# KubiakJakub01/Valle2

Measured on AMD Instinct MI355X. Metric: acoustic tokens/sec (AR decode), higher is better.
Workload: dtype f32; 1 GPU; configs[1]: 12-layer/512-dim AR decoder greedy generate, batch 32, 1024-token prompt -> 512 new tokens, 1xMI355X per rank; rows_per_gpu=32

## Files before the change

### include/valle_hip.h

```cpp
#ifndef VALLE_HIP_H
#define VALLE_HIP_H

#include <stddef.h>
#include <stdint.h>

#ifdef __cplusplus
extern "C" {
#endif

#define VH_VERSION 135
#define VH_MAX_TABLES 32
#define VH_SAMPLE_MAX_V 16384
#define VH_HEAD_DIM 64

enum { VH_OK = 0, VH_EINVAL = -1, VH_EALIGN = -2, VH_EUNSUPPORTED = -3, VH_ELAUNCH = -4,
       VH_ESTATE = -5 };

enum { VH_ACT_NONE = 0, VH_ACT_GELU_ERF = 1,
       VH_ACT_GELU_BWD = 2,
       VH_ACT_GELU_ERF_D = 3,
       VH_ACT_MUL = 4          };

enum {
    VH_MASK_FULL = 0,
    VH_MASK_PREFIX = 1,
    VH_MASK_EXPLICIT = 2
};

int vh_version(void);
const char* vh_last_error(void);

enum { VH_TUNE_DECODE_VARIANT = 0,
       VH_TUNE_DECODE_WAVES = 1,
       VH_TUNE_ROW_GROUPS = 2,
       VH_TUNE_TILE_DMA = 4,
       VH_TUNE_REDUCE_BLOCK = 3,
       VH_TUNE_FFN_FUSED = 5,
       VH_TUNE_GRAPH_STEPS = 6,
       VH_TUNE_FFN_SLICE = 7,
       VH_TUNE_FFN_ROWS = 8,
       VH_TUNE_LN_STATS = 9,
       VH_TUNE_TAIL_SPLIT = 10,
       VH_TUNE_TN_WGS = 11,
       VH_TUNE_DECODE_COMBINE = 12,
       VH_TUNE_ATTN_BWD = 13,
       VH_TUNE_ATTN_BWD_CHUNKS = 14,
       VH_TUNE_BF16_GEMM = 15,
       VH_TUNE_COUNT = 16 };
int vh_set_tuning(int knob, int value);

typedef struct { uint64_t seed; uint64_t site; float p; } vh_dropout_spec;
int vh_dropout(const float* x, int ldx, float* out, int ldo, int64_t rows, int cols, const vh_dropout_spec* spec,
               void* stream);
int vh_dropout_mask(uint8_t* keep, int64_t rows, int cols, const vh_dropout_spec* spec, void* stream);

enum { VH_DEVERR_EMBED_ID = 1, VH_DEVERR_TARGET = 2 };
int vh_embed_sum_pe(const int64_t* ids, int64_t ids_bstride, int64_t ids_tstride,
                    int64_t ids_jstride, const float* const* tables, const int32_t* vocab, int n_tables,
                    const float* pe, int pos0, const int32_t* lens, float* out,
                    int64_t out_bstride, int out_t0, int B, int T, int d, int32_t* err_flag,
                    const int32_t* row_pos0, const int32_t* row_t0, const vh_dropout_spec* drop, void* stream);

int vh_add_pe(const float* x, const float* pe, float* out, int B, int T, int d, int pos0, void* stream);

int vh_layernorm(const float* x, const float* gamma, const float* beta, const float* ada_scale,
                 const float* ada_shift, float* out, int rows, int d, float eps, void* stream);

int vh_linear(const float* A, int lda, const float* W, const float* bias, const float* residual,
              int ldr, float* out, int ldo, int M, int N, int K, int act, const float* ln_gamma,
              const float* ln_beta, const float* ada_scale, const float* ada_shift, float ln_eps,
              void* stream);

size_t vh_linear_ws_bytes(int M, int N, int K);
int vh_linear_ws(const float* A, int lda, const float* W, const float* bias, const float* residual,
                 int ldr, float* out, int ldo, int M, int N, int K, int act, void* workspace,
                 size_t workspace_bytes, void* stream);

int vh_linear_qkv(const float* A, int lda, const float* Wqkv, float* q_out, int ldq, float* kcache,
                  float* vcache, const int32_t* cache_len, int B, int T, int d_model, int n_heads,
                  int S_max, const float* ln_gamma, const float* ln_beta, const float* ada_scale,
                  const float* ada_shift, float ln_eps, void* stream);
// ... 150 lines not shown
    float *x;
    float *q, *attn, *hidden, *logits;
    void *attn_partial;
    void *gemm_ws;
    size_t gemm_ws_bytes;
    int32_t *cache_len, *audio_pos, *eos_count;
    const int32_t *pos_base;
    int64_t *codes;
    int64_t codes_stride;
    int top_k;
    float top_p, temperature;
    uint64_t seed;
    float *sum_logprobs;
    void *ffn_ws;
    size_t ffn_ws_bytes;
    int kv_bf16;
    int prefix_len, prefix_S;
    size_t attn_partial_bytes;
    void *head_ws;
    size_t head_ws_bytes;
    const uint64_t *seed_dev;
    const uint16_t *proj_w16;
    int n_groups, beams_per_group, prefix_cap;
    const int32_t *prefix_lens;
    const vh_row_sampling *row_sampling;
} vh_ar_decoder_desc;

typedef struct vh_ar_decoder vh_ar_decoder;
vh_ar_decoder* vh_ar_decoder_create(const vh_ar_decoder_desc* desc);
void vh_ar_decoder_destroy(vh_ar_decoder* dec);
int vh_ar_decoder_step(vh_ar_decoder* dec, void* stream);
int vh_ar_decoder_capture(vh_ar_decoder* dec, void* stream);
int vh_ar_decoder_replay(vh_ar_decoder* dec, int n_steps, void* stream);
int vh_ar_decoder_profile_attn(vh_ar_decoder* dec, int n_steps, void* stream, float* mean_ms,
                               float* floor_ms, float* kernel_ms);

int vh_layernorm_bwd(const float* x, const float* gamma, const float* beta, const float* ada_scale,
                     const float* dy, float* dx, float* dgamma, float* dbeta, float* dscale,
                     float* dshift, const float* dres, float* dcolsum, float* dx_drop, const vh_dropout_spec* drop,
                     int rows, int d, float eps, void* stream);
int vh_gelu(const float* pre, const float* dh, float* out, int64_t n, void* stream);
int vh_softmax_rows(float* S, int ld, int B, int n_heads, int Tq, int Tk, float scale, int mode,
                    int x_len, const int32_t* x_len_dev, const int32_t* kv_len, const uint8_t* mask,
                    const uint8_t* pad, void* stream);
int vh_softmax_bwd(const float* P, float* dP, int ld, int64_t rows, int Tk, float scale, void* stream);
int vh_cross_entropy(const float* logits, int ld, int V, const int64_t* target, float* loss,
                     float* dlogits, int ldd, int rows, int32_t* err_flag, void* stream);
int vh_embed_bwd(const int64_t* ids, int64_t ids_bstride, int64_t ids_tstride, const float* dout,
                 int64_t dout_bstride, int out_t0, float* dtable, int vocab, int B, int T, int d,
                 int32_t* err_flag, const vh_dropout_spec* drop, void* stream);
int vh_colsum(const float* x, int ld, float* out, int rows, int cols, void* stream);

typedef struct { const float* w; const float* b; float* dw; float* db; } vh_adaproj_item;
int vh_adaproj_fwd(const vh_adaproj_item* items, int n, const float* emb, float* out, int N, int K, void* stream);
int vh_adaproj_bwd(const vh_adaproj_item* items, int n, const float* emb, const float* dout, float* demb, int N, int K,
                   void* stream);

int vh_categorical_rows(const float* logits, int ld, int V, int rows, float temperature, int greedy,
                        uint64_t seed, uint32_t stream_id, int64_t* tokens, int64_t tokens_stride,
                        float* logprob, void* stream);

size_t vh_adamw_ws_bytes(void);
int vh_adamw_flat(float* param, float* grad, float* exp_avg, float* exp_avg_sq, int64_t n, float lr,
                  float beta1, float beta2, float eps, float weight_decay, int step, float grad_scale,
                  float max_norm, int zero_grad, void* workspace, float* norm_out, const int32_t* block_slot,
                  const int32_t* slot_step, const int32_t* guard, void* stream);

size_t vh_linear_ex_ws_bytes(int M, int N, int K);
int vh_linear_ex(const float* A, int lda, const float* W, const float* bias, const float* residual, int ldr,
                 float* out, int ldo, float* pre_out, int ldp, float* dcolsum, int M, int N, int K, int act,
                 const vh_dropout_spec* drop, void* workspace, size_t workspace_bytes, void* stream);

int vh_transpose(const float* in, int ldi, int rows, int cols, float* out, int ldo, void* stream);
typedef struct { const float* in; float* out; int32_t ldi, rows, cols, ldo, tile0, pad_; } vh_transpose_item;
int vh_transpose_many(const vh_transpose_item* items, int n, int total_tiles, void* stream);

size_t vh_gemm_tn_ws_bytes(int M, int NI, int NJ);
int vh_gemm_tn(const float* A, int lda, const float* B, int ldb, float* C, int ldc, int M, int NI, int NJ,
               void* workspace, size_t workspace_bytes, void* stream);

int vh_gemm_batched(const float* A, int lda, int64_t sAb, int64_t sAh, int a_kmajor, const float* B,
                    int ldb, int64_t sBb, int64_t sBh, int b_kmajor, float* C, int ldc, int64_t sCb,
                    int64_t sCh, int M, int N, int K, int batch, int H, int k_splits, void* stream);

typedef struct {
    int B, T, d_model, n_heads, dff, n_layers, S_max, mode, x_len;
    float ln_eps;
    const vh_layer* layers;
    const float* ada;
    const int32_t *x_len_dev, *kv_len;
    const uint8_t *mask, *pad;
    float *x, *xn, *q, *attn, *hidden;
    void *gemm_ws;
    size_t gemm_ws_bytes;
    const float *x_in;
} vh_forward_desc;
int vh_transformer_forward(const vh_forward_desc* desc, void* stream);

int vh_h16_format(void);
int vh_to_bf16(const float* src, int64_t lds, uint16_t* dst, int64_t ldd, int64_t rows, int cols, void* stream);
int vh_layernorm_bf16(const float* x, const float* gamma, const float* beta, const float* ada_scale,
                      const float* ada_shift, uint16_t* out, int rows, int d, float eps, void* stream);
int vh_linear_bf16(const uint16_t* A, int lda, const uint16_t* W, const float* bias, const float* residual, int ldr,
                   void* out, int ldo, int out_bf16, int M, int N, int K, int act, void* stream);
int vh_linear_qkv_bf16(const uint16_t* A, int lda, const uint16_t* Wqkv, uint16_t* q_out, int ldq, uint16_t* kcache16,
                       uint16_t* vcache16, const int32_t* cache_len, int B, int T, int d_model, int n_heads, int S_max,
                       void* stream);
int vh_attn_rows_bf16(const uint16_t* q, int ldq, const uint16_t* kcache16, const uint16_t* vcache16, uint16_t* out, int ldo,
                      int B, int n_heads, int Tq, int Tk, int S_max, int mode, int x_len, const int32_t* x_len_dev,
                      const int32_t* kv_len, void* stream);

typedef struct { const uint16_t *wqkv, *wo, *w1, *w2; uint16_t *kcache16, *vcache16; } vh_layer16;
typedef struct {
    int B, T, d_model, n_heads, dff, n_layers, S_max, mode, x_len;
    float ln_eps;
    const vh_layer* layers;
    const vh_layer16* layers16;
    const float* ada;
    const int32_t *x_len_dev, *kv_len;
    float* x;
    const float* x_in;
    uint16_t *xn16, *q16, *attn16, *hidden16;
} vh_forward16_desc;
int vh_transformer_forward_bf16(const vh_forward16_desc* desc, void* stream);

#ifdef __cplusplus
}
#endif
// ... 2 lines not shown
```

### valle2_amd/_lib.py

```python
from __future__ import annotations

import ctypes as C
import os
from pathlib import Path

import torch

_HERE = Path(__file__).resolve().parent
LIB_PATH = _HERE / 'csrc' / 'libvalle_hip.so'

c_f32p = C.c_void_p
c_i32p = C.c_void_p
c_i64p = C.c_void_p
c_u8p = C.c_void_p


class VhError(RuntimeError):
    pass


class VhDropoutSpec(C.Structure):
    _fields_ = [('seed', C.c_uint64), ('site', C.c_uint64), ('p', C.c_float)]


# ... 12 lines not shown
        'wqkv_f16', 'wo16', 'w1_f16', 'w2_16')]


class VhArDecoderDesc(C.Structure):
    _fields_ = [
        ('B', C.c_int), ('d_model', C.c_int), ('n_heads', C.c_int), ('dff', C.c_int),
        ('n_layers', C.c_int), ('S_max', C.c_int), ('V', C.c_int), ('eos', C.c_int),
        ('n_split', C.c_int), ('ln_eps', C.c_float),
        ('layers', C.POINTER(VhLayer)),
        ('proj_w', C.c_void_p), ('audio_emb', C.c_void_p), ('audio_pe', C.c_void_p),
        ('x', C.c_void_p), ('q', C.c_void_p), ('attn', C.c_void_p), ('hidden', C.c_void_p),
        ('logits', C.c_void_p), ('attn_partial', C.c_void_p), ('gemm_ws', C.c_void_p),
        ('gemm_ws_bytes', C.c_size_t),
        ('cache_len', C.c_void_p), ('audio_pos', C.c_void_p), ('eos_count', C.c_void_p),
        ('pos_base', C.c_void_p), ('codes', C.c_void_p), ('codes_stride', C.c_int64),
        ('top_k', C.c_int), ('top_p', C.c_float), ('temperature', C.c_float), ('seed', C.c_uint64),
        ('sum_logprobs', C.c_void_p), ('ffn_ws', C.c_void_p), ('ffn_ws_bytes', C.c_size_t), ('kv_bf16', C.c_int),
        ('prefix_len', C.c_int), ('prefix_S', C.c_int), ('attn_partial_bytes', C.c_size_t),
        ('head_ws', C.c_void_p), ('head_ws_bytes', C.c_size_t), ('seed_dev', C.c_void_p), ('proj_w16', C.c_void_p),
        ('n_groups', C.c_int), ('beams_per_group', C.c_int), ('prefix_cap', C.c_int), ('prefix_lens', C.c_void_p),
        ('row_sampling', C.c_void_p),
    ]


class VhForwardDesc(C.Structure):
    _fields_ = [
        ('B', C.c_int), ('T', C.c_int), ('d_model', C.c_int), ('n_heads', C.c_int),
        ('dff', C.c_int), ('n_layers', C.c_int), ('S_max', C.c_int), ('mode', C.c_int),
        ('x_len', C.c_int), ('ln_eps', C.c_float),
        ('layers', C.POINTER(VhLayer)), ('ada', C.c_void_p),
        ('x_len_dev', C.c_void_p), ('kv_len', C.c_void_p), ('mask', C.c_void_p), ('pad', C.c_void_p),
        ('x', C.c_void_p), ('xn', C.c_void_p), ('q', C.c_void_p), ('attn', C.c_void_p),
        ('hidden', C.c_void_p), ('gemm_ws', C.c_void_p), ('gemm_ws_bytes', C.c_size_t), ('x_in', C.c_void_p),
    ]


class VhLayer16(C.Structure):
    _fields_ = [(n, C.c_void_p) for n in ('wqkv', 'wo', 'w1', 'w2', 'kcache16', 'vcache16')]


class VhForward16Desc(C.Structure):
    _fields_ = [
        ('B', C.c_int), ('T', C.c_int), ('d_model', C.c_int), ('n_heads', C.c_int),
        ('dff', C.c_int), ('n_layers', C.c_int), ('S_max', C.c_int), ('mode', C.c_int),
        ('x_len', C.c_int), ('ln_eps', C.c_float),
        ('layers', C.POINTER(VhLayer)), ('layers16', C.POINTER(VhLayer16)), ('ada', C.c_void_p),
        ('x_len_dev', C.c_void_p), ('kv_len', C.c_void_p), ('x', C.c_void_p), ('x_in', C.c_void_p),
        ('xn16', C.c_void_p), ('q16', C.c_void_p), ('attn16', C.c_void_p), ('hidden16', C.c_void_p),
    ]


SIGNATURES = {
    'vh_version': (C.c_int, []),
    'vh_last_error': (C.c_char_p, []),
    'vh_set_tuning': (C.c_int, [C.c_int, C.c_int]),
    'vh_embed_sum_pe': (C.c_int, [c_i64p, C.c_int64, C.c_int64, C.c_int64, C.POINTER(C.c_void_p),
                                  C.POINTER(C.c_int32), C.c_int, c_f32p, C.c_int, c_i32p, c_f32p, C.c_int64,
                                  C.c_int, C.c_int, C.c_int, C.c_int, c_i32p, c_i32p, c_i32p, c_dropp, C.c_void_p]),
    'vh_dropout': (C.c_int, [c_f32p, C.c_int, c_f32p, C.c_int, C.c_int64, C.c_int, c_dropp, C.c_void_p]),
    'vh_dropout_mask': (C.c_int, [c_u8p, C.c_int64, C.c_int, c_dropp, C.c_void_p]),
    'vh_add_pe': (C.c_int, [c_f32p, c_f32p, c_f32p, C.c_int, C.c_int, C.c_int, C.c_int, C.c_void_p]),
    'vh_layernorm': (C.c_int, [c_f32p, c_f32p, c_f32p, c_f32p, c_f32p, c_f32p, C.c_int, C.c_int,
                               C.c_float, C.c_void_p]),
    'vh_linear': (C.c_int, [c_f32p, C.c_int, c_f32p, c_f32p, c_f32p, C.c_int, c_f32p, C.c_int,
                            C.c_int, C.c_int, C.c_int, C.c_int, c_f32p, c_f32p, c_f32p, c_f32p,
                            C.c_float, C.c_void_p]),
# ... 59 lines not shown
    'vh_kv_store': (C.c_int, [c_f32p, C.c_int, c_f32p, c_f32p, C.c_int, C.c_int, C.c_int, C.c_int, C.c_int, C.c_void_p]),
    'vh_greedy_step': (C.c_int, [c_f32p, C.c_int, C.c_int, C.c_int, c_i64p, C.c_int64, c_i32p,
                                 c_i32p, c_f32p, c_f32p, c_i32p, c_i32p, c_f32p, C.c_int, C.c_int,
                                 C.c_void_p]),
    'vh_decode_groups_poll': (C.c_int, [c_i64p, C.c_int64, C.c_int, c_i32p, c_i32p, c_i32p, C.c_int, C.c_int, C.c_int, C.c_int,
                                        c_i32p, c_i32p, c_i32p, C.c_void_p]),
    'vh_decode_group_reset': (C.c_int, [c_i64p, C.c_int64, C.c_int, c_i64p, C.c_int, C.c_int, C.c_int, C.c_int, C.c_int, C.c_int,
                                        C.c_int, c_i32p, c_i32p, c_i32p, c_f32p, c_i32p, C.c_void_p]),
    'vh_head_greedy_ws_bytes': (C.c_size_t, [C.c_int, C.c_int]),
    'vh_head_greedy': (C.c_int, [c_f32p, C.c_int, c_f32p, c_f32p, C.c_int, C.c_int, C.c_int, c_i64p, C.c_int64, c_i32p,
                                 c_i32p, c_f32p, c_f32p, c_i32p, c_i32p, c_f32p, C.c_int, C.c_int, C.c_void_p, C.c_size_t,
                                 C.c_void_p]),
    'vh_sample_step': (C.c_int, [c_f32p, C.c_int, C.c_int, C.c_int, C.c_int, C.c_float, C.c_float, C.c_uint64,
                                 c_i64p, C.c_int64, c_i32p, c_i32p, c_f32p, c_f32p, c_f32p, c_i32p, c_i32p,
                                 c_f32p, C.c_int, C.c_int, C.c_void_p]),
    'vh_sample_step_wide': (C.c_int, [c_f32p, C.c_int, C.c_int, C.c_int, C.c_int, C.c_float, C.c_float, C.c_uint64,
                                      c_i64p, C.c_int64, c_i32p, c_i32p, c_f32p, c_f32p, c_f32p, c_i32p, c_i32p,
                                      c_f32p, C.c_int, C.c_int, C.c_void_p]),
    'vh_sample_step_rows': (C.c_int, [c_f32p, C.c_int, C.c_int, C.c_int, C.c_void_p, c_i64p, C.c_int64, c_i32p, c_i32p,
                                      c_f32p, c_f32p, c_f32p, c_i32p, c_i32p, c_f32p, C.c_int, C.c_int, C.c_void_p]),
    'vh_sample_step_wide_rows': (C.c_int, [c_f32p, C.c_int, C.c_int, C.c_int, C.c_void_p, c_i64p, C.c_int64, c_i32p, c_i32p,
                                           c_f32p, c_f32p, c_f32p, c_i32p, c_i32p, c_f32p, C.c_int, C.c_int, C.c_void_p]),
    'vh_categorical_rows': (C.c_int, [c_f32p, C.c_int, C.c_int, C.c_int, C.c_float, C.c_int, C.c_uint64, C.c_uint32,
                                      c_i64p, C.c_int64, c_f32p, C.c_void_p]),
    'vh_adamw_ws_bytes': (C.c_size_t, []),
    'vh_adamw_flat': (C.c_int, [c_f32p, c_f32p, c_f32p, c_f32p, C.c_int64, C.c_float, C.c_float, C.c_float,
                                C.c_float, C.c_float, C.c_int, C.c_float, C.c_float, C.c_int, C.c_void_p,
                                c_f32p, c_i32p, c_i32p, c_i32p, C.c_void_p]),
    'vh_ar_decoder_create': (C.c_void_p, [C.POINTER(VhArDecoderDesc)]),
    'vh_ar_decoder_destroy': (None, [C.c_void_p]),
    'vh_ar_decoder_step': (C.c_int, [C.c_void_p, C.c_void_p]),
    'vh_ar_decoder_capture': (C.c_int, [C.c_void_p, C.c_void_p]),
    'vh_ar_decoder_replay': (C.c_int, [C.c_void_p, C.c_int, C.c_void_p]),
    'vh_ar_decoder_profile_attn': (C.c_int, [C.c_void_p, C.c_int, C.c_void_p,
                                             C.POINTER(C.c_float), C.POINTER(C.c_float), C.POINTER(C.c_float)]),
    'vh_layernorm_bwd': (C.c_int, [c_f32p, c_f32p, c_f32p, c_f32p, c_f32p, c_f32p, c_f32p, c_f32p, c_f32p,
                                   c_f32p, c_f32p, c_f32p, c_f32p, c_dropp, C.c_int, C.c_int, C.c_float, C.c_void_p]),
    'vh_gelu': (C.c_int, [c_f32p, c_f32p, c_f32p, C.c_int64, C.c_void_p]),
    'vh_softmax_rows': (C.c_int, [c_f32p, C.c_int, C.c_int, C.c_int, C.c_int, C.c_int, C.c_float, C.c_int,
                                  C.c_int, c_i32p, c_i32p, c_u8p, c_u8p, C.c_void_p]),
    'vh_softmax_bwd': (C.c_int, [c_f32p, c_f32p, C.c_int, C.c_int64, C.c_int, C.c_float, C.c_void_p]),
    'vh_cross_entropy': (C.c_int, [c_f32p, C.c_int, C.c_int, c_i64p, c_f32p, c_f32p, C.c_int, C.c_int,
                                   c_i32p, C.c_void_p]),
    'vh_embed_bwd': (C.c_int, [c_i64p, C.c_int64, C.c_int64, c_f32p, C.c_int64, C.c_int, c_f32p, C.c_int,
                               C.c_int, C.c_int, C.c_int, c_i32p, c_dropp, C.c_void_p]),
    'vh_colsum': (C.c_int, [c_f32p, C.c_int, c_f32p, C.c_int, C.c_int, C.c_void_p]),
    'vh_linear_ex': (C.c_int, [c_f32p, C.c_int, c_f32p, c_f32p, c_f32p, C.c_int, c_f32p, C.c_int, c_f32p, C.c_int,
                               c_f32p, C.c_int, C.c_int, C.c_int, C.c_int, c_dropp, C.c_void_p, C.c_size_t, C.c_void_p]),
    'vh_linear_ex_ws_bytes': (C.c_size_t, [C.c_int, C.c_int, C.c_int]),
    'vh_transpose': (C.c_int, [c_f32p, C.c_int, C.c_int, C.c_int, c_f32p, C.c_int, C.c_void_p]),
    'vh_transpose_many': (C.c_int, [C.c_void_p, C.c_int, C.c_int, C.c_void_p]),
    'vh_adaproj_fwd': (C.c_int, [C.c_void_p, C.c_int, c_f32p, c_f32p, C.c_int, C.c_int, C.c_void_p]),
    'vh_adaproj_bwd': (C.c_int, [C.c_void_p, C.c_int, c_f32p, c_f32p, c_f32p, C.c_int, C.c_int, C.c_void_p]),
    'vh_gemm_tn_ws_bytes': (C.c_size_t, [C.c_int, C.c_int, C.c_int]),
    'vh_gemm_tn': (C.c_int, [c_f32p, C.c_int, c_f32p, C.c_int, c_f32p, C.c_int, C.c_int, C.c_int, C.c_int,
                             C.c_void_p, C.c_size_t, C.c_void_p]),
    'vh_gemm_batched': (C.c_int, [c_f32p, C.c_int, C.c_int64, C.c_int64, C.c_int, c_f32p, C.c_int, C.c_int64,
                                  C.c_int64, C.c_int, c_f32p, C.c_int, C.c_int64, C.c_int64, C.c_int, C.c_int,
                                  C.c_int, C.c_int, C.c_int, C.c_int, C.c_void_p]),
    'vh_transformer_forward': (C.c_int, [C.POINTER(VhForwardDesc), C.c_void_p]),
    'vh_h16_format': (C.c_int, []),
    'vh_to_bf16': (C.c_int, [c_f32p, C.c_int64, C.c_void_p, C.c_int64, C.c_int64, C.c_int, C.c_void_p]),
    'vh_layernorm_bf16': (C.c_int, [c_f32p, c_f32p, c_f32p, c_f32p, c_f32p, C.c_void_p, C.c_int, C.c_int, C.c_float,
                                    C.c_void_p]),
    'vh_linear_bf16': (C.c_int, [C.c_void_p, C.c_int, C.c_void_p, c_f32p, c_f32p, C.c_int, C.c_void_p, C.c_int, C.c_int,
                                 C.c_int, C.c_int, C.c_int, C.c_int, C.c_void_p]),
    'vh_linear_qkv_bf16': (C.c_int, [C.c_void_p, C.c_int, C.c_void_p, C.c_void_p, C.c_int, C.c_void_p, C.c_void_p, c_i32p,
                                     C.c_int, C.c_int, C.c_int, C.c_int, C.c_int, C.c_void_p]),
    'vh_attn_rows_bf16': (C.c_int, [C.c_void_p, C.c_int, C.c_void_p, C.c_void_p, C.c_void_p, C.c_int, C.c_int, C.c_int,
                                    C.c_int, C.c_int, C.c_int, C.c_int, C.c_int, c_i32p, c_i32p, C.c_void_p]),
    'vh_transformer_forward_bf16': (C.c_int, [C.POINTER(VhForward16Desc), C.c_void_p]),
}

_lib = None


def load_library(path: os.PathLike | None = None) -> C.CDLL:
    p = Path(path or LIB_PATH)
    if not p.exists():
        raise VhError(f'{p} not found: build it with `python __graft_entry__.py build` '
                      f'(make -C valle2_amd/csrc). There is no CPU fallback.')
    lib = C.CDLL(str(p))
    for name, (res, args) in SIGNATURES.items():
        fn = getattr(lib, name)
        fn.restype = res
        fn.argtypes = args
    raw_set = lib.vh_set_tuning

    def set_tuning(knob, value):
        global TUNING_EPOCH
        TUNING_EPOCH += 1
        return raw_set(knob, value)
    lib.vh_set_tuning = set_tuning
    return lib


TUNING_EPOCH = 0


def h16_dtype():
    global _H16
    if _H16 is None:
        _H16 = torch.bfloat16 if load_library().vh_h16_format() else torch.float16
    return _H16


_H16 = None


def lib() -> C.CDLL:
    global _lib
    if _lib is None:
        if not torch.cuda.is_available():
            raise VhError('valle2_amd needs a HIP device (MI355X): torch.cuda.is_available() is '
                          'False and there is no CPU fallback. The CPU oracle lives in oracle/ and '
                          'is test infrastructure only.')
        _lib = load_library()
        n = sum(1 for line in open('/proc/self/maps') if 'libamdhip64' in line and ' r-xp ' in line)
        if n > 1:
            raise VhError('two HIP runtimes are mapped in this process; import torch before '
                          'loading libvalle_hip.so')
    return _lib


def check(rc: int, what: str = ''):
    if rc != 0:
        msg = lib().vh_last_error()
        raise VhError(f'{what} failed ({rc}): {msg.decode() if msg else ""}')


# ... 85 lines not shown
```

### valle2_amd/csrc/attention.hip

```cpp
#include <hip/hip_ext.h>
#include "vh_common.h"
#include <mutex>
#include <queue>
#include <type_traits>
#include <unordered_map>
#include <vector>

#define HD VH_HEAD_DIM
#define LOG2E 1.44269504088896340736f
#define NEG_INF (-INFINITY)

#define PART_LD 72

typedef uint32_t u32x4 __attribute__((ext_vector_type(4)));
__device__ __forceinline__ u32x4 ld16_stream(const uint16_t* p) {
    return __builtin_nontemporal_load(reinterpret_cast<const u32x4*>(p));
}
__device__ __forceinline__ float row8_sum(float v) {
    v += dpp_get<0xB1, 0xF>(v, 0.f);
    v += dpp_get<0x4E, 0xF>(v, 0.f);
    v += dpp_get<0x141, 0xF>(v, 0.f);
    return v;
}
#define BF_LO(w) vh_h16_lo(w)
// ... 465 lines not shown
    const bool fused_combine = n_split > 1 && (combine_knob == 1 || (combine_knob == 0 && n_split == 2));
    unsigned* arrived = fused_combine ? (unsigned*)((char*)partial + decode_records_bytes(B, n_heads, n_split)) : nullptr;
    if (variant != 1 && big && n_split == 1 && nw == 0) {
        const int waves = 8;
        hipExtLaunchKernelGGL((attn_decode_ring_kernel<8, 2>), grid, dim3(waves * 64), 0, s, g_attn_ev[0], g_attn_ev[1], 0, q,
                              ldq, kcache, vcache, out, ldo, cache_len, len_bias, n_heads, S_max);
    } else {
        const int waves = nw ? nw : (big ? 16 : 4);
        if (waves == 16) AD(attn_decode_kernel, 16); else if (waves == 8) AD(attn_decode_kernel, 8);
        else AD(attn_decode_kernel, 4);
    }
#undef AD
    if (n_split > 1 && !fused_combine)
        hipLaunchKernelGGL(attn_decode_combine_kernel, dim3(B * n_heads), dim3(64), 0, s,
                           (const float*)partial, out, ldo, n_heads, n_split);
    VH_CHECK_LAUNCH("vh_attn_decode");
    return VH_OK;
}

#define QB 128
#define KT 32
#define KLD 68

struct RowsArgs {
    const float* q; int ldq;
    const float* kc; const float* vc;
    float* out; int ldo;
    int n_heads, Tq, Tk, S_max, mode, x_len;
    const int32_t* x_len_dev; const int32_t* kv_len;
    const uint8_t* mask; const uint8_t* pad;
    int n_qblocks;
    float* lse2;
    int64_t mask_bstride;
};

__global__ __launch_bounds__(256, 2) void attn_rows_kernel(RowsArgs a) {
    __shared__ __attribute__((aligned(16))) float lds[2 * 2 * KT * KLD];
    const int tid = threadIdx.x, lane = tid & 63, w = tid >> 6;
    const int r = lane & 31, h = lane >> 5;
    const int n_bh = gridDim.x / a.n_qblocks;
    const int bh = blockIdx.x % n_bh, b = bh / a.n_heads, head = bh - b * a.n_heads;
    const int q0 = (a.n_qblocks - 1 - (int)(blockIdx.x / n_bh)) * QB;
    const int q_off = a.Tk - a.Tq;
    const int kvl = a.kv_len ? min(a.kv_len[b], a.Tk) : a.Tk;
    const int xl = a.x_len_dev ? a.x_len_dev[b] : a.x_len;

    const int last_pos = q_off + min(q0 + QB, a.Tq) - 1;
    int kmax = kvl;
    if (a.mode == VH_MASK_PREFIX) kmax = min(kvl, max(xl, last_pos >= xl ? last_pos + 1 : 0));
    if (a.mode == VH_MASK_EXPLICIT) kmax = a.Tk;
    const int n_tiles = (kmax + KT - 1) / KT;

    const int qi = q0 + w * 32 + r;
    const int qpos = q_off + qi;
    const float qscale = 0.125f * LOG2E;
    f32x4 qf[8];
    {
        const float* qp = a.q + ((int64_t)b * a.Tq + qi) * a.ldq + head * HD + 4 * h;
#pragma unroll
        for (int t = 0; t < 8; ++t)
            qf[t] = qi < a.Tq ? ld4(qp + 8 * t) * qscale : f32x4{0.f, 0.f, 0.f, 0.f};
    }

    const float* kb = a.kc + (int64_t)bh * a.S_max * HD;
    const float* vb = a.vc + (int64_t)bh * a.S_max * HD;
    const int skey = tid >> 4, squad = (tid & 15) * 4;
    f32x4 rk[2], rv[2];
    auto gload = [&](int k0) {
#pragma unroll
        for (int i = 0; i < 2; ++i) {
            const uint32_t off = (uint32_t)(min(k0 + skey + 16 * i, a.Tk - 1) * HD + squad) * 4u;
            rk[i] = ld4((const float*)((const char*)kb + off));
            rv[i] = ld4((const float*)((const char*)vb + off));
        }
    };
// ... 84 lines not shown
            }
#pragma unroll
            for (int e = 0; e < 16; ++e) {
                const float* vrow = vs + ((e & 3) + 8 * (e >> 2) + 4 * h) * KLD + r;
                O0 = __builtin_amdgcn_mfma_f32_32x32x2f32(vrow[0], S[e], O0, 0, 0, 0);
                O1 = __builtin_amdgcn_mfma_f32_32x32x2f32(vrow[32], S[e], O1, 0, 0, 0);
            }
        }
        if (kt + 1 < n_tiles) lstore(cur ^ 1);
        __syncthreads();
    }

    const float ltot = l + __shfl_xor(l, 32, 64);
    const float inv = 1.0f / ltot;
    if (a.lse2 && h == 0 && qi < a.Tq) a.lse2[(int64_t)bh * a.Tq + qi] = m + log2f(ltot);
    float* ob = lds;
#pragma unroll
    for (int g4 = 0; g4 < 4; ++g4) {
        f32x4 v0 = {O0[4 * g4], O0[4 * g4 + 1], O0[4 * g4 + 2], O0[4 * g4 + 3]};
        f32x4 v1 = {O1[4 * g4], O1[4 * g4 + 1], O1[4 * g4 + 2], O1[4 * g4 + 3]};
        st4(ob + (w * 32 + r) * KLD + 8 * g4 + 4 * h, v0 * inv);
        st4(ob + (w * 32 + r) * KLD + 32 + 8 * g4 + 4 * h, v1 * inv);
    }
    __syncthreads();
#pragma unroll
    for (int i = 0; i < 8; ++i) {
        const int row = skey + 16 * i;
        if (q0 + row < a.Tq)
            st4(a.out + ((int64_t)b * a.Tq + q0 + row) * a.ldo + head * HD + squad,
                ld4(ob + row * KLD + squad));
    }
}

static int attn_rows_launch(const float* q, int ldq, const float* kcache, const float* vcache,
                            float* out, int ldo, int B, int n_heads, int Tq, int Tk, int S_max,
                            int mode, int x_len, const int32_t* x_len_dev, const int32_t* kv_len,
                            const uint8_t* mask, const uint8_t* pad, float* lse2, void* stream, int64_t mask_bstride = 0) {
    VH_REQUIRE(q && kcache && vcache && out, VH_EINVAL, "vh_attn_rows: null pointer");
    VH_REQUIRE(B >= 0 && n_heads > 0 && Tq >= 0 && Tk >= Tq && S_max >= Tk, VH_EINVAL,
               "vh_attn_rows: bad dims B=%d h=%d Tq=%d Tk=%d S_max=%d", B, n_heads, Tq, Tk, S_max);
    VH_REQUIRE(mode == VH_MASK_FULL || mode == VH_MASK_PREFIX || mode == VH_MASK_EXPLICIT, VH_EINVAL,
               "vh_attn_rows: mode=%d", mode);
    VH_REQUIRE(mode != VH_MASK_EXPLICIT || mask, VH_EINVAL, "vh_attn_rows: explicit mode needs mask");
    VH_REQUIRE(ldq % 4 == 0 && ldo % 4 == 0 && ldq >= n_heads * HD && ldo >= n_heads * HD, VH_EINVAL,
               "vh_attn_rows: ldq=%d ldo=%d", ldq, ldo);
    VH_REQUIRE(vh_aligned16(q) && vh_aligned16(kcache) && vh_aligned16(vcache) && vh_aligned16(out),
               VH_EALIGN, "vh_attn_rows: pointers must be 16-byte aligned");
    if (B == 0 || Tq == 0) return VH_OK;
    const int nqb = (Tq + QB - 1) / QB;
    RowsArgs a{q, ldq, kcache, vcache, out, ldo, n_heads, Tq, Tk, S_max, mode, x_len,
               x_len_dev, kv_len, mask, pad, nqb, lse2, mask_bstride};
    dim3 grid(nqb * B * n_heads);
    hipLaunchKernelGGL(attn_rows_kernel, grid, dim3(256), 0, (hipStream_t)stream, a);
    VH_CHECK_LAUNCH("vh_attn_rows");
    return VH_OK;
}

extern "C" int vh_attn_rows(const float* q, int ldq, const float* kcache, const float* vcache,
                            float* out, int ldo, int B, int n_heads, int Tq, int Tk, int S_max,
                            int mode, int x_len, const int32_t* x_len_dev, const int32_t* kv_len,
                            const uint8_t* mask, const uint8_t* pad, void* stream) {
    return attn_rows_launch(q, ldq, kcache, vcache, out, ldo, B, n_heads, Tq, Tk, S_max, mode, x_len,
                            x_len_dev, kv_len, mask, pad, nullptr, stream);
}

extern "C" int vh_attn_rows_bmask(const float* q, int ldq, const float* kcache, const float* vcache, float* out, int ldo, int B,
                                  int n_heads, int Tq, int Tk, int S_max, const uint8_t* mask, int64_t mask_batch_stride,
                                  const uint8_t* pad, void* stream) {
    VH_REQUIRE(mask && (mask_batch_stride == 0 || mask_batch_stride >= (int64_t)Tq * Tk), VH_EINVAL,
               "vh_attn_rows_bmask: a (B,Tq,Tk) mask with batch stride >= Tq*Tk (or 0: one mask for every row), got %lld",
               (long long)mask_batch_stride);
    return attn_rows_launch(q, ldq, kcache, vcache, out, ldo, B, n_heads, Tq, Tk, S_max, VH_MASK_EXPLICIT, 0, nullptr, nullptr,
                            mask, pad, nullptr, stream, mask_batch_stride);
}

extern "C" int vh_attn_rows_lse(const float* q, int ldq, const float* kcache, const float* vcache,
                                float* out, int ldo, int B, int n_heads, int Tq, int Tk, int S_max,
                                int mode, int x_len, const int32_t* x_len_dev, const int32_t* kv_len,
                                const uint8_t* mask, const uint8_t* pad, float* lse2, void* stream) {
    VH_REQUIRE(lse2, VH_EINVAL, "vh_attn_rows_lse: null lse2");
    return attn_rows_launch(q, ldq, kcache, vcache, out, ldo, B, n_heads, Tq, Tk, S_max, mode, x_len,
                            x_len_dev, kv_len, mask, pad, lse2, stream);
}

struct BwdArgs {
    const float* q; int ldq;
    const float* kc; const float* vc;
    const float* o; int ldo;
// ... 1020 lines not shown
```

### valle2_amd/csrc/elementwise.hip

```cpp
#include "vh_common.h"

template <int CAP>
struct TablePtrs {
    const float* t[CAP];
    int vocab[CAP];
};

template <int CAP>
__global__ __launch_bounds__(256) void embed_sum_pe_kernel(
    const int64_t* __restrict__ ids, int64_t ids_bs, int64_t ids_ts, int64_t ids_js, TablePtrs<CAP> tabs,
    int n_tables, const float* __restrict__ pe, int pos0, const int32_t* __restrict__ lens,
    float* __restrict__ out, int64_t out_bs, int out_t0, int T, int d, int32_t* __restrict__ err_flag,
    const int32_t* __restrict__ row_pos0, const int32_t* __restrict__ row_t0, DropArgs drop) {
    const int lane = threadIdx.x & 63;
    const int t = blockIdx.x * 4 + (threadIdx.x >> 6);
    const int b = blockIdx.y;
    if (t >= T) return;
    if (lens && t >= lens[b]) return;
    if (row_pos0) pos0 = row_pos0[b];
    if (row_t0) out_t0 = row_t0[b];
    const int64_t* idp = ids + b * ids_bs + t * ids_ts;
    int64_t row[CAP];
    bool bad = false;
    for (int j = 0; j < n_tables; ++j) {
// ... 216 lines not shown
            if (ada_scale) y = ld4(ada_scale + c) * y + ld4(ada_shift + c);
            st4(orow + c, y);
        }
    }
}

extern "C" int vh_layernorm(const float* x, const float* gamma, const float* beta,
                            const float* ada_scale, const float* ada_shift, float* out, int rows,
                            int d, float eps, void* stream) {
    VH_REQUIRE(x && gamma && beta && out, VH_EINVAL, "vh_layernorm: null pointer");
    VH_REQUIRE((ada_scale == nullptr) == (ada_shift == nullptr), VH_EINVAL,
               "vh_layernorm: ada_scale and ada_shift must be given together");
    VH_REQUIRE(rows >= 0 && d > 0 && d % 4 == 0 && d <= 4096, VH_EINVAL,
               "vh_layernorm: bad dims rows=%d d=%d (d multiple of 4, <= 4096)", rows, d);
    VH_REQUIRE(vh_aligned16(x) && vh_aligned16(out) && vh_aligned16(gamma) && vh_aligned16(beta) &&
                   vh_aligned16(ada_scale) && vh_aligned16(ada_shift),
               VH_EALIGN, "vh_layernorm: pointers must be 16-byte aligned");
    if (rows == 0) return VH_OK;
    dim3 grid((rows + 3) / 4), block(256);
    hipStream_t s = (hipStream_t)stream;
#define LN_LAUNCH(NV)                                                                            \
    hipLaunchKernelGGL(layernorm_kernel<NV>, grid, block, 0, s, x, gamma, beta, ada_scale,       \
                       ada_shift, out, rows, d, eps)
    if (d <= 256) LN_LAUNCH(1);
    else if (d <= 512) LN_LAUNCH(2);
    else if (d <= 1024) LN_LAUNCH(4);
    else if (d <= 2048) LN_LAUNCH(8);
    else LN_LAUNCH(16);
#undef LN_LAUNCH
    VH_CHECK_LAUNCH("vh_layernorm");
    return VH_OK;
}

__global__ __launch_bounds__(256) void greedy_step_kernel(
    const float* __restrict__ logits, int ldl, int V, int eos, int64_t* __restrict__ codes,
    int64_t codes_stride, int32_t* __restrict__ eos_count, const int32_t* __restrict__ pos_base,
    const float* __restrict__ audio_emb, const float* __restrict__ pe,
    int32_t* __restrict__ audio_pos, int32_t* __restrict__ cache_len, float* __restrict__ x_next, int d) {
    __shared__ float s_val[4];
    __shared__ int s_idx[4];
    __shared__ int s_tok;
    const int b = blockIdx.x;
    const int tid = threadIdx.x, lane = tid & 63, w = tid >> 6;
    const float* lr = logits + (int64_t)b * ldl;
    float best = -INFINITY;
    int bi = 0x7fffffff;
    for (int i = tid; i < V; i += 256) {
        const float v = lr[i];
        if (v > best || (v == best && i < bi)) { best = v; bi = i; }
    }
#pragma unroll
    for (int o = 32; o > 0; o >>= 1) {
        const float ov = __shfl_xor(best, o, 64);
        const int oi = __shfl_xor(bi, o, 64);
        if (ov > best || (ov == best && oi < bi)) { best = ov; bi = oi; }
    }
    if (lane == 0) { s_val[w] = best; s_idx[w] = bi; }
    __syncthreads();
    const int pos = audio_pos[b];
    if (tid == 0) {
        for (int k = 1; k < 4; ++k)
            if (s_val[k] > best || (s_val[k] == best && s_idx[k] < bi)) { best = s_val[k]; bi = s_idx[k]; }
        int64_t* row = codes + (int64_t)b * codes_stride;
        int tok = bi;
        if (row[pos - 1] == (int64_t)eos) tok = eos;
        row[pos] = tok;
        if (tok == eos) atomicAdd(&eos_count[pos - (pos_base ? pos_base[b] : 0)], 1);
        s_tok = tok;
    }
    __syncthreads();
    const int tok = s_tok;
    const float* er = audio_emb + (int64_t)tok * d;
    const float* pr = pe + (int64_t)pos * d;
    for (int c = tid * 4; c < d; c += 1024) {
        const f32x4 e = ld4(er + c) + ld4(pr + c);
        st4(x_next + (int64_t)b * d + c, e);
    }
    if (tid == 0) {
        audio_pos[b] = pos + 1;
        cache_len[b] += 1;
    }
}

extern "C" int vh_greedy_step(const float* logits, int ldl, int V, int eos, int64_t* codes,
                              int64_t codes_stride, int32_t* eos_count, const int32_t* pos_base,
                              const float* audio_emb, const float* pe, int32_t* audio_pos,
                              int32_t* cache_len, float* x_next, int B, int d, void* stream) {
    VH_REQUIRE(logits && codes && eos_count && audio_emb && pe && audio_pos && cache_len && x_next,
               VH_EINVAL, "vh_greedy_step: null pointer");
    VH_REQUIRE(B > 0 && V > 0 && ldl >= V && d > 0 && d % 4 == 0, VH_EINVAL,
               "vh_greedy_step: bad dims B=%d V=%d ldl=%d d=%d", B, V, ldl, d);
    VH_REQUIRE(vh_aligned16(audio_emb) && vh_aligned16(pe) && vh_aligned16(x_next), VH_EALIGN,
               "vh_greedy_step: audio_emb/pe/x_next must be 16-byte aligned");
    hipLaunchKernelGGL(greedy_step_kernel, dim3(B), dim3(256), 0, (hipStream_t)stream, logits, ldl,
                       V, eos, codes, codes_stride, eos_count, pos_base, audio_emb, pe, audio_pos,
                       cache_len, x_next, d);
    VH_CHECK_LAUNCH("vh_greedy_step");
    return VH_OK;
}

#define SAMPLE_MAXV 2048

__device__ __forceinline__ float uniform01(uint64_t seed, uint32_t row, uint32_t pos) {
    uint64_t z = seed + 0x9E3779B97F4A7C15ull * (((uint64_t)row << 32) | (uint64_t)(pos + 1u));
    z = (z ^ (z >> 30)) * 0xBF58476D1CE4E5B9ull;
    z = (z ^ (z >> 27)) * 0x94D049BB133111EBull;
    z ^= z >> 31;
    return (float)(z >> 40) * (1.0f / 16777216.0f);
}

__device__ __forceinline__ uint32_t okey(float x) {
    const uint32_t u = __float_as_uint(x);
    return (u & 0x80000000u) ? ~u : (u | 0x80000000u);
}

#define ROW_SAMPLING_LOAD(rec)                                            \
    do {                                                                  \
        const vh_row_sampling r_ = (rec);                                 \
        seed = r_.seed;                                                   \
        draw_key = r_.key;                                                \
        top_k = r_.top_k;                                                 \
        top_p = r_.top_p;                                                 \
        inv_temp = 1.0f / r_.temperature;                                 \
        greedy = top_k == 1;                                              \
        if (greedy) { top_p = 1.0f; inv_temp = 1.0f; }                    \
    } while (0)

__global__ __launch_bounds__(256) void sample_step_kernel(
    const float* __restrict__ logits, int ldl, int V, int eos, int top_k, float top_p, float inv_temp,
    uint64_t seed, int64_t* __restrict__ codes, int64_t codes_stride, int32_t* __restrict__ eos_count,
    const int32_t* __restrict__ pos_base, float* __restrict__ sum_logprobs,
    const float* __restrict__ audio_emb, const float* __restrict__ pe, int32_t* __restrict__ audio_pos,
    int32_t* __restrict__ cache_len, float* __restrict__ x_next, int d, int npow2, const uint64_t* __restrict__ seed_dev,
    const vh_row_sampling* __restrict__ rs) {
    uint32_t draw_key = blockIdx.x;
    bool greedy = false;
    if (rs) {
        ROW_SAMPLING_LOAD(rs[blockIdx.x]);
    } else if (seed_dev) {
        seed += *seed_dev;
    }
    __shared__ float s_val[SAMPLE_MAXV];
    __shared__ int s_idx[SAMPLE_MAXV];
    __shared__ int s_hist[256];
    __shared__ int s_sel[4];
    __shared__ float s_red[8];
    __shared__ int s_tok;
    const int b = blockIdx.x, tid = threadIdx.x, lane = tid & 63, wv = tid >> 6;
    const float* lr = logits + (int64_t)b * ldl;
    const int pos = audio_pos[b];
    int pick_tok = 0;
    float pick_logprob = 0.f;

    const bool fast = top_k > 0 && top_k < V && top_p == 1.0f;
    if (fast) {
        float vmax = -INFINITY;
        for (int i = tid; i < V; i += 256) {
            float x = lr[i] * inv_temp;
            if (greedy) x += 0.0f;
            s_val[i] = x;
            vmax = fmaxf(vmax, x);
        }
        vmax = wave_max(vmax);
        if (lane == 0) s_red[wv] = vmax;
        uint32_t prefix = 0, mask = 0;
        int want = top_k;
        for (int shift = 24; shift >= 0; shift -= 8) {
// ... 118 lines not shown
                float tail = 0.f;
                int n2 = n_keep;
                while (n2 > 1) {
                    tail += expf(s_val[n2 - 1] - m);
                    if (tail > limit) break;
                    --n2;
                }
                n_keep = n2;
                total = 0.f;
                for (int i = 0; i < n_keep; ++i) total += expf(s_val[i] - m);
            }
            const float u = uniform01(seed, draw_key, (uint32_t)pos) * total;
            float acc = 0.f;
            int pick = n_keep - 1;
            for (int i = 0; i < n_keep; ++i) {
                acc += expf(s_val[i] - m);
                if (acc > u) { pick = i; break; }
            }
            s_sel[2] = s_idx[pick];
            s_red[4] = (s_val[pick] - m) - logf(total);
        }
        __syncthreads();
        pick_tok = s_sel[2];
        pick_logprob = s_red[4];
    }
    if (greedy) pick_logprob = 0.f;
    if (tid == 0) {
        int64_t* row = codes + (int64_t)b * codes_stride;
        int tok = pick_tok;
        const bool finished = row[pos - 1] == (int64_t)eos;
        if (sum_logprobs && !finished) sum_logprobs[b] += pick_logprob;
        if (finished) tok = eos;
        row[pos] = tok;
        if (tok == eos) atomicAdd(&eos_count[pos - (pos_base ? pos_base[b] : 0)], 1);
        s_tok = tok;
    }
    __syncthreads();
    const int tok = s_tok;
    const float* er = audio_emb + (int64_t)tok * d;
    const float* pr = pe + (int64_t)pos * d;
    for (int c = tid * 4; c < d; c += 1024) {
        const f32x4 e = ld4(er + c) + ld4(pr + c);
        st4(x_next + (int64_t)b * d + c, e);
    }
    if (tid == 0) {
        audio_pos[b] = pos + 1;
        cache_len[b] += 1;
    }
}

int vh_internal_sample_step(const float* logits, int ldl, int V, int eos, int top_k, float top_p,
                            float temperature, uint64_t seed, const uint64_t* seed_dev, const vh_row_sampling* rs, int64_t* codes, int64_t codes_stride,
                            int32_t* eos_count, const int32_t* pos_base, float* sum_logprobs,
                            const float* audio_emb, const float* pe, int32_t* audio_pos,
                            int32_t* cache_len, float* x_next, int B, int d, void* stream) {
    VH_REQUIRE(logits && codes && eos_count && audio_emb && pe && audio_pos && cache_len && x_next,
               VH_EINVAL, "vh_sample_step: null pointer");
    VH_REQUIRE(B > 0 && V > 0 && V <= SAMPLE_MAXV && ldl >= V && d > 0 && d % 4 == 0, VH_EINVAL,
               "vh_sample_step: bad dims B=%d V=%d (<= %d) ldl=%d d=%d", B, V, SAMPLE_MAXV, ldl, d);
    VH_REQUIRE(rs || temperature > 0.f, VH_EINVAL, "vh_sample_step: temperature must be positive");
    VH_REQUIRE(vh_aligned16(rs), VH_EALIGN, "vh_sample_step: the per-row sampling records must be 16-byte aligned");
    VH_REQUIRE(vh_aligned16(audio_emb) && vh_aligned16(pe) && vh_aligned16(x_next), VH_EALIGN,
               "vh_sample_step: audio_emb/pe/x_next must be 16-byte aligned");
    int npow2 = 2;
    while (npow2 < V) npow2 <<= 1;
    hipLaunchKernelGGL(sample_step_kernel, dim3(B), dim3(256), 0, (hipStream_t)stream, logits, ldl, V,
                       eos, top_k, top_p, rs ? 1.0f : 1.0f / temperature, seed, codes, codes_stride, eos_count,
                       pos_base, sum_logprobs, audio_emb, pe, audio_pos, cache_len, x_next, d, npow2, seed_dev, rs);
    VH_CHECK_LAUNCH("vh_sample_step");
    return VH_OK;
}

extern "C" int vh_sample_step(const float* logits, int ldl, int V, int eos, int top_k, float top_p,
                              float temperature, uint64_t seed, int64_t* codes, int64_t codes_stride,
                              int32_t* eos_count, const int32_t* pos_base, float* sum_logprobs,
                              const float* audio_emb, const float* pe, int32_t* audio_pos,
                              int32_t* cache_len, float* x_next, int B, int d, void* stream) {
    return vh_internal_sample_step(logits, ldl, V, eos, top_k, top_p, temperature, seed, nullptr, nullptr, codes, codes_stride, eos_count,
                                   pos_base, sum_logprobs, audio_emb, pe, audio_pos, cache_len, x_next, B, d, stream);
}

extern "C" int vh_sample_step_rows(const float* logits, int ldl, int V, int eos, const vh_row_sampling* rs, int64_t* codes,
                                  int64_t codes_stride, int32_t* eos_count, const int32_t* pos_base, float* sum_logprobs,
                                  const float* audio_emb, const float* pe, int32_t* audio_pos, int32_t* cache_len,
                                  float* x_next, int B, int d, void* stream) {
    VH_REQUIRE(rs, VH_EINVAL, "vh_sample_step_rows: null sampling records (vh_sample_step takes one filter for every row)");
    return vh_internal_sample_step(logits, ldl, V, eos, 0, 1.f, 1.f, 0, nullptr, rs, codes, codes_stride, eos_count, pos_base, sum_logprobs,
                                  audio_emb, pe, audio_pos, cache_len, x_next, B, d, stream);
}

#define WIDE_THREADS 1024
#define WIDE_WAVES (WIDE_THREADS / 64)
#define WIDE_PER (VH_SAMPLE_MAX_V / WIDE_THREADS)

template <typename T>
__device__ __forceinline__ T wide_block_scan(T v, T* s_w, T* excl, T* total) {
    const int lane = threadIdx.x & 63, wv = threadIdx.x >> 6;
    T incl = v;
#pragma unroll
    for (int o = 1; o < 64; o <<= 1) {
        const T up = __shfl_up(incl, o, 64);
// ... 15 lines not shown
    return before + incl;
}

__device__ __forceinline__ void wide_draw(const float* s_val, int n, float m, float u01, float* s_w, int* s_out,
                                          float* s_tot) {
    const int tid = threadIdx.x;
    const int per = (n + WIDE_THREADS - 1) / WIDE_THREADS;
    const int j0 = min(n, tid * per), j1 = min(n, j0 + per);
    float s = 0.f;
    for (int j = j0; j < j1; ++j) s += expf(s_val[j] - m);
    if (tid == 0) s_out[0] = n - 1;
    float excl, total;
    const float incl = wide_block_scan(s, s_w, &excl, &total);
    const float u = u01 * total;
    if (j1 > j0 && excl <= u && incl > u) {
        float acc = excl;
        int pick = j1 - 1;
        for (int j = j0; j < j1; ++j) {
            acc += expf(s_val[j] - m);
            if (acc > u) { pick = j; break; }
        }
        s_out[0] = pick;
    }
    if (tid == 0) s_tot[0] = total;
    __syncthreads();
}

__global__ __launch_bounds__(WIDE_THREADS) void sample_step_wide_kernel(
    const float* __restrict__ logits, int ldl, int V, int eos, int top_k, float top_p, float inv_temp,
    uint64_t seed, int64_t* __restrict__ codes, int64_t codes_stride, int32_t* __restrict__ eos_count,
    const int32_t* __restrict__ pos_base, float* __restrict__ sum_logprobs,
    const float* __restrict__ audio_emb, const float* __restrict__ pe, int32_t* __restrict__ audio_pos,
    int32_t* __restrict__ cache_len, float* __restrict__ x_next, int d, const uint64_t* __restrict__ seed_dev,
    const vh_row_sampling* __restrict__ rs) {
    uint32_t draw_key = blockIdx.x;
    bool greedy = false;
    if (rs) {
        ROW_SAMPLING_LOAD(rs[blockIdx.x]);
    } else if (seed_dev) {
        seed += *seed_dev;
    }
    __shared__ float s_val[VH_SAMPLE_MAX_V];
    __shared__ int s_idx[VH_SAMPLE_MAX_V];
    __shared__ int s_hist[256];
    __shared__ float s_wf[WIDE_WAVES];
    __shared__ int s_wi[WIDE_WAVES];
    __shared__ float s_max[WIDE_WAVES];
    __shared__ int s_sel[3];
    __shared__ float s_tot;
    __shared__ int s_tok;
    const int b = blockIdx.x, tid = threadIdx.x, lane = tid & 63, wv = tid >> 6;
    const float* lr = logits + (int64_t)b * ldl;
    const int pos = audio_pos[b];

    float vmax = -INFINITY;
    for (int i = tid; i < V; i += WIDE_THREADS) {
        float x = lr[i] * inv_temp;
        if (greedy) x += 0.0f;
        s_val[i] = x;
        vmax = fmaxf(vmax, x);
    }
    vmax = wave_max(vmax);
    if (lane == 0) s_max[wv] = vmax;
    __syncthreads();
    float m = s_max[0];
#pragma unroll
    for (int w = 1; w < WIDE_WAVES; ++w) m = fmaxf(m, s_max[w]);
// ... 98 lines not shown
            }
        int n_keep = n;
        if (top_p >= 0.f && top_p <= 1.f) {
            const int run = (n + WIDE_THREADS - 1) / WIDE_THREADS;
            const int j1 = max(0, n - tid * run), j0 = max(0, j1 - run);
            float s = 0.f;
            for (int j = j1 - 1; j >= j0; --j) s += expf(s_val[j] - m);
            float after, total;
            wide_block_scan(s, s_wf, &after, &total);
            const float limit = (1.0f - top_p) * total;
            float tail = after;
            int over = 0;
            for (int j = j1 - 1; j >= j0; --j) {
                tail += expf(s_val[j] - m);
                over += j >= 1 && tail > limit;
            }
            int ex, n_over;
            wide_block_scan(over, s_wi, &ex, &n_over);
            n_keep = 1 + n_over;
        }
        wide_draw(s_val, n_keep, m, u01, s_wf, &s_sel[2], &s_tot);
    }
    const int slot = s_sel[2];
    const int pick_tok = s_idx[slot];
    const float pick_logprob = greedy ? 0.f : (s_val[slot] - m) - logf(s_tot);

    if (tid == 0) {
        int64_t* row = codes + (int64_t)b * codes_stride;
        int tok = pick_tok;
        const bool finished = row[pos - 1] == (int64_t)eos;
        if (sum_logprobs && !finished) sum_logprobs[b] += pick_logprob;
        if (finished) tok = eos;
        row[pos] = tok;
        if (tok == eos) atomicAdd(&eos_count[pos - (pos_base ? pos_base[b] : 0)], 1);
        s_tok = tok;
    }
    __syncthreads();
    const int tok = s_tok;
    const float* er = audio_emb + (int64_t)tok * d;
    const float* pr = pe + (int64_t)pos * d;
    for (int c = tid * 4; c < d; c += 4 * WIDE_THREADS) {
        const f32x4 e = ld4(er + c) + ld4(pr + c);
        st4(x_next + (int64_t)b * d + c, e);
    }
    if (tid == 0) {
        audio_pos[b] = pos + 1;
        cache_len[b] += 1;
    }
}

int vh_internal_sample_step_wide(const float* logits, int ldl, int V, int eos, int top_k, float top_p,
                                 float temperature, uint64_t seed, const uint64_t* seed_dev, const vh_row_sampling* rs, int64_t* codes,
                                 int64_t codes_stride, int32_t* eos_count, const int32_t* pos_base, float* sum_logprobs,
                                 const float* audio_emb, const float* pe, int32_t* audio_pos,
                                 int32_t* cache_len, float* x_next, int B, int d, void* stream) {
    VH_REQUIRE(logits && codes && eos_count && audio_emb && pe && audio_pos && cache_len && x_next,
               VH_EINVAL, "vh_sample_step_wide: null pointer");
    VH_REQUIRE(B > 0 && V > 0 && V <= VH_SAMPLE_MAX_V && ldl >= V && d > 0 && d % 4 == 0, VH_EINVAL,
               "vh_sample_step_wide: bad dims B=%d V=%d (<= %d) ldl=%d d=%d", B, V, VH_SAMPLE_MAX_V, ldl, d);
    VH_REQUIRE(rs || temperature > 0.f, VH_EINVAL, "vh_sample_step_wide: temperature must be positive");
    VH_REQUIRE(vh_aligned16(rs), VH_EALIGN, "vh_sample_step_wide: the per-row sampling records must be 16-byte aligned");
    VH_REQUIRE(vh_aligned16(audio_emb) && vh_aligned16(pe) && vh_aligned16(x_next), VH_EALIGN,
               "vh_sample_step_wide: audio_emb/pe/x_next must be 16-byte aligned");
    hipLaunchKernelGGL(sample_step_wide_kernel, dim3(B), dim3(WIDE_THREADS), 0, (hipStream_t)stream, logits, ldl, V,
                       eos, top_k, top_p, rs ? 1.0f : 1.0f / temperature, seed, codes, codes_stride, eos_count,
                       pos_base, sum_logprobs, audio_emb, pe, audio_pos, cache_len, x_next, d, seed_dev, rs);
    VH_CHECK_LAUNCH("vh_sample_step_wide");
    return VH_OK;
}

extern "C" int vh_sample_step_wide(const float* logits, int ldl, int V, int eos, int top_k, float top_p,
                                   float temperature, uint64_t seed, int64_t* codes, int64_t codes_stride,
                                   int32_t* eos_count, const int32_t* pos_base, float* sum_logprobs,
                                   const float* audio_emb, const float* pe, int32_t* audio_pos,
                                   int32_t* cache_len, float* x_next, int B, int d, void* stream) {
    return vh_internal_sample_step_wide(logits, ldl, V, eos, top_k, top_p, temperature, seed, nullptr, nullptr, codes, codes_stride,
                                        eos_count, pos_base, sum_logprobs, audio_emb, pe, audio_pos, cache_len, x_next, B, d,
                                        stream);
}

extern "C" int vh_sample_step_wide_rows(const float* logits, int ldl, int V, int eos, const vh_row_sampling* rs, int64_t* codes,
                                       int64_t codes_stride, int32_t* eos_count, const int32_t* pos_base, float* sum_logprobs,
                                       const float* audio_emb, const float* pe, int32_t* audio_pos, int32_t* cache_len,
                                       float* x_next, int B, int d, void* stream) {
    VH_REQUIRE(rs, VH_EINVAL, "vh_sample_step_wide_rows: null sampling records (vh_sample_step_wide takes one filter for every row)");
    return vh_internal_sample_step_wide(logits, ldl, V, eos, 0, 1.f, 1.f, 0, nullptr, rs, codes, codes_stride, eos_count, pos_base, sum_logprobs,
                                       audio_emb, pe, audio_pos, cache_len, x_next, B, d, stream);
}


__global__ __launch_bounds__(256) void categorical_rows_kernel(
    const float* __restrict__ logits, int ld, int V, int rows, float inv_temp, int greedy, uint64_t seed,
    uint32_t stream_id, int64_t* __restrict__ tokens, int64_t tokens_stride, float* __restrict__ logprob) {
    const int lane = threadIdx.x & 63;
    const int row = blockIdx.x * 4 + (threadIdx.x >> 6);
    if (row >= rows) return;
    const float* lr = logits + (int64_t)row * ld;
    const int chunk = (V + 63) / 64;
    const int i0 = min(V, lane * chunk), i1 = min(V, i0 + chunk);
// ... 185 lines not shown
```

### valle2_amd/csrc/gemm.hip

```cpp
#include <type_traits>

#include "vh_common.h"

struct GemmArgs {
    const float* A;
    int lda;
    const float* W;
    const float* bias;
    const float* res;
    int ldr;
    float* out;
    int ldo;
    int M, N, K, act;
    float* kc;
    float* vc;
    const int32_t* cache_len;
    int T, S_max, d_model, n_heads;
    float* aux;
    int ldx;
    float* colsum;
    int k_len;
    int rg_rows;
    int w16;
    DropArgs drop;
// ... 3 lines not shown
#endif
};

#ifdef VH_STAMPS
#define STAMP(k)                                                                         \
    do {                                                                                 \
        if (a.dbg && (threadIdx.x & 63) == 0)                                            \
            a.dbg[((int64_t)blockIdx.x * 16 + (threadIdx.x >> 6)) * 8 + (k)] = wall_clock64(); \
    } while (0)
#else
#define STAMP(k)
#endif

enum { EPI_PLAIN = 0, EPI_QKV = 1, EPI_PARTIAL = 2,
       EPI_QKV16 = 3 ,
       EPI_HEAD = 4  ,
       EPI_QKV_HD = 5  };
#define IS_QKV(E) ((E) == EPI_QKV || (E) == EPI_QKV16 || (E) == EPI_QKV_HD)

struct HeadStep {
    uint64_t* cand;
    int* counters;
    int V, eos;
    int64_t* codes;
    int64_t codes_stride;
    int32_t* eos_count;
    const int32_t* pos_base;
    const float* audio_emb;
    const float* pe;
    int32_t* audio_pos;
    int32_t* cache_len;
    float* x_next;
    int d;
};

__device__ __forceinline__ uint32_t vh_bf16_bits(float x) {
    const uint32_t u = __float_as_uint(x);
    return (u + 0x7fffu + ((u >> 16) & 1u)) >> 16;
}

template <int EPI>
__device__ __forceinline__ void store4(const GemmArgs& a, int m, int n, f32x4 v) {
    if (m >= a.M || n >= a.N) return;
    if (EPI == EPI_PARTIAL) {
        st4(a.out + ((int64_t)blockIdx.y * a.M + m) * a.ldo + n, v);
        return;
    }
    if (EPI == EPI_QKV) {
        const int which = n / a.d_model, c = n - which * a.d_model;
        if (which == 0) {
            st4(a.out + (int64_t)m * a.ldo + c, v);
        } else {
            const int head = c / VH_HEAD_DIM, e = c - head * VH_HEAD_DIM;
            const int b = m / a.T, t = m - b * a.T;
            const int pos = (a.cache_len ? a.cache_len[b] : 0) + t;
            float* base = which == 1 ? a.kc : a.vc;
            st4(base + (((int64_t)b * a.n_heads + head) * a.S_max + pos) * VH_HEAD_DIM + e, v);
        }
        return;
    }
    if (EPI == EPI_QKV_HD) {
        const int which = n / a.d_model, c = n - which * a.d_model;
        if (which == 0) {
            st4(a.out + (int64_t)m * a.ldo + c, v);
        } else {
            const int head = c / a.head_dim, e = c - head * a.head_dim;
// ... 278 lines not shown
                else if (a.act == VH_ACT_MUL) sv *= a.res[(int64_t)m * a.ldr + en + j];
                else if (a.res) sv += a.res[(int64_t)m * a.ldr + en + j];
                a.out[(int64_t)m * a.ldo + en + j] = sv;
            }
        }
    }
    if (EPI == EPI_PLAIN && a.colsum) tile_colsum(a, ct, csum, n0, tid);
}

template <int EPI>
__global__ __launch_bounds__(256, 2) void gemm_tile_kernel(GemmArgs a, int tiles_m, int tiles_n) {
    __shared__ __attribute__((aligned(16))) float lds[2][2][TM * LDS_LD];
    const int tid = threadIdx.x, lane = tid & 63, w = tid >> 6;
    const int r = lane & 31, h = lane >> 5;
    const int wm = w >> 1, wn = w & 1;

    const int nwg = tiles_m * tiles_n;
    const int bid = blockIdx.x;
    const int q8 = nwg / 8, r8 = nwg % 8, xcd = bid % 8;
    const int tile = (xcd < r8 ? xcd * (q8 + 1) : r8 * (q8 + 1) + (xcd - r8) * q8) + bid / 8;
    const int m0 = (tile / tiles_n) * TM, n0 = (tile % tiles_n) * TN;

    const int srow = tid >> 3, skq = (tid & 7) * 4;
    f32x4 ra[4], rw[4];
    const float* pa[4];
    const float* pw[4];
#pragma unroll
    for (int i = 0; i < 4; ++i) {
        const int row = srow + 32 * i;
        pa[i] = a.A + (int64_t)min(m0 + row, a.M - 1) * a.lda + skq + blockIdx.y * a.k_len;
        pw[i] = a.W + (int64_t)min(n0 + row, a.N - 1) * a.K + skq + blockIdx.y * a.k_len;
    }
    auto gload1 = [&](int i, int k0) {
        const int kk = k0 + skq < a.k_len ? k0 : 0;
        ra[i] = ld4(pa[i] + kk);
        rw[i] = ld4(pw[i] + kk);
    };
    auto gload = [&](int k0) {
#pragma unroll
        for (int i = 0; i < 4; ++i) gload1(i, k0);
    };
    auto lstore = [&](int buf, int k0) {
        const bool kin = k0 + skq < a.k_len;
#pragma unroll
        for (int i = 0; i < 4; ++i) {
            const int row = srow + 32 * i;
            st4(&lds[buf][0][row * LDS_LD + skq], kin ? ra[i] : f32x4{0.f, 0.f, 0.f, 0.f});
            st4(&lds[buf][1][row * LDS_LD + skq], kin ? rw[i] : f32x4{0.f, 0.f, 0.f, 0.f});
        }
    };

    f32x16 acc[2][2];
#pragma unroll
    for (int i = 0; i < 2; ++i)
#pragma unroll
        for (int j = 0; j < 2; ++j)
#pragma unroll
            for (int e = 0; e < 16; ++e) acc[i][j][e] = 0.f;

    const int nk = (a.k_len + TK - 1) / TK;
    gload(0);
    lstore(0, 0);

    TileEpi epi;
    tile_prefetch<EPI>(a, m0, n0, tid, epi);
    __syncthreads();
    f32x4 fa[2][2], fw[2][2];
// ... 15 lines not shown
            if (t < 3) fload((t + 1) & 1, cur, t + 1);
            __builtin_amdgcn_sched_barrier(0);
#pragma unroll
            for (int j = 0; j < 4; ++j) {
                acc[0][0] = __builtin_amdgcn_mfma_f32_32x32x2f32(fa[t & 1][0][j], fw[t & 1][0][j], acc[0][0], 0, 0, 0);
                acc[0][1] = __builtin_amdgcn_mfma_f32_32x32x2f32(fa[t & 1][0][j], fw[t & 1][1][j], acc[0][1], 0, 0, 0);
                acc[1][0] = __builtin_amdgcn_mfma_f32_32x32x2f32(fa[t & 1][1][j], fw[t & 1][0][j], acc[1][0], 0, 0, 0);
                acc[1][1] = __builtin_amdgcn_mfma_f32_32x32x2f32(fa[t & 1][1][j], fw[t & 1][1][j], acc[1][1], 0, 0, 0);
            }
            __builtin_amdgcn_sched_barrier(0);
        }
        if constexpr (PF) lstore(cur ^ 1, (kt + 1) * TK);
        __syncthreads();
        if constexpr (PF) fload(0, cur ^ 1, 0);
    };
    for (int kt = 0; kt + 1 < nk; ++kt) kstep(kt, std::true_type{});
    kstep(nk - 1, std::false_type{});

    tile_prefetch_late<EPI>(a, m0, n0, tid, epi);
    tile_epilogue<EPI>(a, acc, &lds[0][0][0], m0, n0, tid, epi);
}

#ifdef VH_TILE_PROBE
__device__ long long vh_tile_probe[8192 * 4 * 200];
__device__ unsigned vh_tile_hwid[8192 * 2];
#define VH_TP(ev, step) do { if (lane == 0) tp[(ev) * 64 + (step)] = clock64(); } while (0)
#else
#define VH_TP(ev, step) do { } while (0)
#endif

struct TailSplit {
    int n_whole, split, k_len;
    float* ws;
};

template <int EPI, bool DROP = false>
__global__ __launch_bounds__(256, 2) void gemm_tile_dma_kernel(GemmArgs a, int tiles_m, int tiles_n, TailSplit ts) {
    __shared__ __attribute__((aligned(16))) float lds[2][2][TM * LDS_LD];
    __builtin_amdgcn_s_setprio(3);
    const int tid = threadIdx.x, lane = tid & 63, w = tid >> 6;
#ifdef VH_TILE_PROBE
    const long long t_entry = clock64();
#endif
    const int r = lane & 31, h = lane >> 5;
    const int wm = w >> 1, wn = w & 1;

    const int nwg = ts.n_whole;
    const int bid = blockIdx.x;
    const bool tail = bid >= nwg;
    const int q8 = nwg / 8, r8 = nwg % 8, xcd = bid % 8;
    const int unit = bid - nwg;
    const int tile = tail ? nwg + unit / ts.split
                          : (xcd < r8 ? xcd * (q8 + 1) : r8 * (q8 + 1) + (xcd - r8) * q8) + bid / 8;
    const int m0 = (tile / tiles_n) * TM, n0 = (tile % tiles_n) * TN;
    const int k_len = tail ? ts.k_len : a.k_len;
    const int k_ofs = tail ? (unit % ts.split) * ts.k_len : blockIdx.y * a.k_len;

    const int ws = __builtin_amdgcn_readfirstlane(w);
    const char* baseA = (const char*)(a.A + (int64_t)m0 * a.lda + k_ofs);
    const char* baseW = (const char*)(a.W + (int64_t)n0 * a.K + k_ofs);
    uint32_t voff[8];
#pragma unroll
    for (int i = 0; i < 8; ++i) {
        const int q = ws * 8 + i, row = (q & 15) * 8 + (lane >> 3);
        const int c = (lane & 7) ^ ((row >> 1) & 7);
        voff[i] = q < 16 ? (uint32_t)(min(row, a.M - 1 - m0) * a.lda + 4 * c) * 4u
                         : (uint32_t)(min(row, a.N - 1 - n0) * a.K + 4 * c) * 4u;
    }
    auto dma1 = [&](int i, int buf, int k0) {
        const int q = ws * 8 + i;
        const char* base = (q < 16 ? baseA : baseW) + (int64_t)k0 * 4;
        const uint32_t dst = (uint32_t)(uintptr_t)&lds[buf][q >> 4][(q & 15) * 8 * 32];
        asm volatile("s_mov_b32 m0, %0\n\ts_nop 0\n\tglobal_load_lds_dwordx4 %1, %2"
                     :: "s"(dst), "v"(voff[i]), "s"(base) : "memory");
    };

    f32x16 acc[2][2];
#pragma unroll
    for (int i = 0; i < 2; ++i)
#pragma unroll
        for (int j = 0; j < 2; ++j)
#pragma unroll
            for (int e = 0; e < 16; ++e) acc[i][j][e] = 0.f;

    const int nk = k_len / TK;
#pragma unroll
    for (int i = 0; i < 8; ++i) dma1(i, 0, 0);
// ... 509 lines not shown
    if constexpr (EPI == EPI_HEAD) {
        static_assert(MT == 1 && NW == 8, "head + greedy step: 16 rows x 32 threads");
        __shared__ int s_ticket, s_tok[16], s_pos[16];
        asm volatile("s_waitcnt vmcnt(0)" ::: "memory");
        __syncthreads();
        if (tid == 0) s_ticket = __hip_atomic_fetch_add(hs->counters + blockIdx.z, 1, __ATOMIC_ACQ_REL, __HIP_MEMORY_SCOPE_AGENT);
        __syncthreads();
        if (s_ticket != (int)gridDim.x - 1) return;
        if (tid == 0) hs->counters[blockIdx.z] = 0;
        const int row = tid >> 5, j = tid & 31;
        float bv = -INFINITY;
        int bi = 0x7fffffff;
        if (row < a.M)
            for (int c = j; c < (int)gridDim.x; c += 32) {
                const uint64_t p = __hip_atomic_load(hs->cand + (int64_t)(hr0 + row) * gridDim.x + c, __ATOMIC_RELAXED,
                                                     __HIP_MEMORY_SCOPE_AGENT);
                const float v = __uint_as_float((uint32_t)(p >> 32));
                const int idx = (int)(uint32_t)p;
                if (v > bv || (v == bv && idx < bi)) { bv = v; bi = idx; }
            }
#pragma unroll
        for (int o = 16; o > 0; o >>= 1) {
            const float ov = __shfl_xor(bv, o, 64);
            const int oi = __shfl_xor(bi, o, 64);
            if (ov > bv || (ov == bv && oi < bi)) { bv = ov; bi = oi; }
        }
        if (j == 0 && row < a.M) {
            const int b = hr0 + row;
            const int pos = hs->audio_pos[b];
            int64_t* crow = hs->codes + (int64_t)b * hs->codes_stride;
            int tok = min(bi, hs->V - 1);
            if (crow[pos - 1] == (int64_t)hs->eos) tok = hs->eos;
            crow[pos] = tok;
            if (tok == hs->eos) atomicAdd(&hs->eos_count[pos - (hs->pos_base ? hs->pos_base[b] : 0)], 1);
            s_tok[row] = tok;
            s_pos[row] = pos;
            hs->audio_pos[b] = pos + 1;
            hs->cache_len[b] += 1;
        }
        __syncthreads();
        const int q4 = hs->d >> 2;
        for (int c = tid; c < a.M * q4; c += NW * 64) {
            const int r = c / q4, cc = (c - r * q4) * 4;
            st4(hs->x_next + (int64_t)(hr0 + r) * hs->d + cc,
                ld4(hs->audio_emb + (int64_t)s_tok[r] * hs->d + cc) + ld4(hs->pe + (int64_t)s_pos[r] * hs->d + cc));
        }
    }
}


template <int MT, int NW, int EPI, int PW, int LN, int NJ, bool W16 = false>
__global__ __launch_bounds__(NW * 64) void gemm_skinny_fast(const float* hA, const float* hW, int h_lda, int hK, int h_klen,
                                                            int hM, int hN, GemmArgs a, LnFuse ln) {
    a.A = hA; a.W = hW; a.lda = h_lda; a.K = hK; a.k_len = h_klen; a.M = hM; a.N = hN;
    skinny_body<MT, NW, EPI, PW, LN, NJ, W16>(a, ln);
}

template <int PW>
__global__ __launch_bounds__(512) void gemm_head_greedy_kernel(const float* hA, const float* hW, int h_lda, int hK, int h_klen,
                                                               int hM, int hN, GemmArgs a, HeadStep hs) {
    a.A = hA; a.W = hW; a.lda = h_lda; a.K = hK; a.k_len = h_klen; a.M = hM; a.N = hN;
    LnFuse none{};
    skinny_body<1, 8, EPI_HEAD, PW, 0, 1>(a, none, &hs);
}
__global__ __launch_bounds__(256) void splitk_reduce_kernel(const float* __restrict__ slabs, int n_split,
                                                            GemmArgs a, int lds_) {
    const int idx = blockIdx.x * blockDim.x + threadIdx.x;
// ... 86 lines not shown
}

extern "C" size_t vh_linear_ex_ws_bytes(int M, int N, int K) {
    int n_whole;
    const int split = tail_plan(M, N, K, &n_whole);
    const int tiles = ((M + TM - 1) / TM) * ((N + TN - 1) / TN);
    return split ? (size_t)(tiles - n_whole) * split * TM * TN * sizeof(float) : 0;
}

static bool folded_wide_k(int K) {
    return K > 1024 && K <= 4096 && K % (K <= 2048 ? 256 : 512) == 0;
}

static int splitk_plan(int M, int N, int K) {
    if (M > 64) {
        const int tiles = ((M + TM - 1) / TM) * ((N + TN - 1) / TN);
        if (tiles > 256 || K < 1024) return 0;
        int splits = 1;
        while (splits < 8 && tiles * splits * 2 <= 512 && K % (splits * 2 * TK) == 0 && K / (splits * 2) >= 256) splits *= 2;
        return splits >= 2 ? splits : 0;
    }
    if (K <= 1024 || K % 256 != 0) return 0;
    const int tiles = (N + 15) / 16;
    int splits = min(16, 256 / tiles);
    while (splits > 1 && (K % (splits * 256) != 0)) --splits;
    return splits >= 2 ? splits : 0;
}

extern "C" size_t vh_linear_ws_bytes(int M, int N, int K) {
    const int splits = splitk_plan(M, N, K);
    if (splits) return (size_t)splits * M * ((N + 3) / 4 * 4) * sizeof(float);
    return M > 64 ? vh_linear_ex_ws_bytes(M, N, K) : 0;
}

static int check_gemm(const char* name, const GemmArgs& a, const LnFuse& ln) {
    VH_REQUIRE(a.A && a.W && a.out, VH_EINVAL, "%s: null pointer", name);
    VH_REQUIRE(a.M >= 0 && a.N > 0 && a.K > 0, VH_EINVAL, "%s: bad dims M=%d N=%d K=%d", name, a.M,
               a.N, a.K);
    VH_REQUIRE(a.K % 16 == 0, VH_EUNSUPPORTED, "%s: K=%d must be a multiple of 16", name, a.K);
    VH_REQUIRE(a.lda % 4 == 0 && a.lda >= a.K, VH_EALIGN, "%s: lda=%d", name, a.lda);
    VH_REQUIRE(vh_aligned16(a.A) && vh_aligned16(a.W) && vh_aligned16(a.out) &&
                   vh_aligned16(a.bias) && vh_aligned16(a.res),
               VH_EALIGN, "%s: pointers must be 16-byte aligned", name);
    VH_REQUIRE(a.ldo % 4 == 0 && (!a.res || a.ldr % 4 == 0), VH_EALIGN, "%s: ldo/ldr", name);
    VH_REQUIRE((ln.gamma == nullptr) == (ln.beta == nullptr), VH_EINVAL,
               "%s: ln_gamma and ln_beta must be given together", name);
    VH_REQUIRE((ln.ada_scale == nullptr) == (ln.ada_shift == nullptr), VH_EINVAL,
               "%s: ada_scale and ada_shift must be given together", name);
    VH_REQUIRE(!ln.ada_scale || ln.gamma, VH_EINVAL, "%s: ada_* needs ln_gamma/ln_beta", name);
    VH_REQUIRE(!ln.gamma || (a.M <= 64 && a.K <= 1024), VH_EUNSUPPORTED,
               "%s: fused LayerNorm only for M <= 64 and K <= 1024 (M=%d K=%d); run vh_layernorm first",
               name, a.M, a.K);
    VH_REQUIRE(vh_aligned16(ln.gamma) && vh_aligned16(ln.beta) && vh_aligned16(ln.ada_scale) &&
                   vh_aligned16(ln.ada_shift),
               VH_EALIGN, "%s: LayerNorm vectors must be 16-byte aligned", name);
    return VH_OK;
}

#define SKINNY_ARGS(g) (g).A, (g).W, (g).lda, (g).K, (g).k_len, (g).M, (g).N

template <int EPI>
static int launch_gemm(const char* name, const GemmArgs& a, const LnFuse& ln, hipStream_t s, float* tail_ws = nullptr,
                       size_t tail_ws_bytes = 0) {
    if (a.M == 0) return VH_OK;
    const bool train_epi = a.aux != nullptr || a.colsum != nullptr || a.act >= VH_ACT_GELU_BWD || a.drop.thresh != 0;
    if (a.M <= 64 && !train_epi) {
// ... 116 lines not shown
            }
            if (a.K % 1024 == 0) SF_MT(16, 4, 0, 1);
        }
#undef SF_MT
#undef SF
#undef SFB_MT
#undef SFB
        if constexpr (EPI == EPI_QKV16) {
            vh_set_error("%s: bf16 K/V append needs the folded LayerNorm shapes (K in {128,256,512,640,768,896,1024})", name);
            return VH_EUNSUPPORTED;
        } else {
        if (a.w16) { vh_set_error("%s: no 16-bit-weight form of this shape (K=%d)", name, a.K); return VH_EUNSUPPORTED; }
#define SK(MT, NW, CH, LN) \
    hipLaunchKernelGGL((gemm_skinny_kernel<MT, NW, EPI, CH, LN>), grid, dim3(NW * 64), 0, s, a, ln)
        if (has_ln) {
            if (mt == 1) SK(1, 8, 4, true); else if (mt == 2) SK(2, 8, 4, true); else SK(4, 8, 4, true);
        } else if (wide) {
            if (mt == 1) SK(1, 16, 8, false); else if (mt == 2) SK(2, 16, 8, false); else SK(4, 16, 4, false);
        } else {
            if (mt == 1) SK(1, 8, 4, false); else if (mt == 2) SK(2, 8, 4, false); else SK(4, 8, 4, false);
        }
#undef SK
        }
    } else if constexpr (EPI == EPI_QKV16) {
        vh_set_error("%s: bf16 K/V append is the decode path (M <= 64)", name);
        return VH_EUNSUPPORTED;
    } else if constexpr (EPI == EPI_QKV_HD) {
        vh_set_error("%s: the K/V append at a runtime head width is the decode path (M <= 64)", name);
        return VH_EUNSUPPORTED;
    } else {
        if (a.w16) { vh_set_error("%s: 16-bit weights are the decode step's form (M <= 64)", name); return VH_EUNSUPPORTED; }
        const int tm = (a.M + TM - 1) / TM, tn = (a.N + TN - 1) / TN;
        if (a.k_len % TK == 0 && vh_tuning(VH_TUNE_TILE_DMA) != 1) {
            TailSplit ts{tm * tn, 1, a.K, nullptr};
            if constexpr (EPI == EPI_PLAIN) {
                int n_whole;
                const int split = tail_ws ? tail_plan(a.M, a.N, a.K, &n_whole) : 0;
                if (split && tail_ws_bytes >= (size_t)(tm * tn - n_whole) * split * TM * TN * sizeof(float))
                    ts = TailSplit{n_whole, split, a.K / split, tail_ws};
            }
            const int tail = tm * tn - ts.n_whole;
            if (EPI == EPI_PLAIN && a.drop.thresh)
                hipLaunchKernelGGL((gemm_tile_dma_kernel<EPI, EPI == EPI_PLAIN>), dim3(ts.n_whole + tail * ts.split), dim3(256), 0,
                                   s, a, tm, tn, ts);
            else
                hipLaunchKernelGGL((gemm_tile_dma_kernel<EPI>), dim3(ts.n_whole + tail * ts.split), dim3(256), 0, s, a, tm, tn,
                                   ts);
            if (tail) hipLaunchKernelGGL(tile_tail_fixup_kernel, dim3(tail * 4), dim3(256), 0, s, a, ts, tn);
        } else {
            hipLaunchKernelGGL((gemm_tile_kernel<EPI>), dim3(tm * tn), dim3(256), 0, s, a, tm, tn);
        }
    }
    VH_CHECK_LAUNCH(name);
    return VH_OK;
}

extern "C" int vh_linear(const float* A, int lda, const float* W, const float* bias,
                         const float* residual, int ldr, float* out, int ldo, int M, int N, int K,
                         int act, const float* ln_gamma, const float* ln_beta,
                         const float* ada_scale, const float* ada_shift, float ln_eps,
                         void* stream) {
    GemmArgs a{};
    a.A = A; a.lda = lda; a.W = W; a.bias = bias; a.res = residual; a.ldr = ldr; a.out = out;
    a.ldo = ldo; a.M = M; a.N = N; a.K = K; a.act = act; a.k_len = K;
    LnFuse ln{ln_gamma, ln_beta, ada_scale, ada_shift, ln_eps};
    VH_REQUIRE(act == VH_ACT_NONE || act == VH_ACT_GELU_ERF, VH_EINVAL, "vh_linear: act=%d", act);
    VH_REQUIRE(ldo >= N && (!residual || ldr >= N), VH_EINVAL, "vh_linear: ldo/ldr < N");
    if (int rc = check_gemm("vh_linear", a, ln)) return rc;
    return launch_gemm<EPI_PLAIN>("vh_linear", a, ln, (hipStream_t)stream);
}

extern "C" int vh_linear_ex(const float* A, int lda, const float* W, const float* bias, const float* residual,
                            int ldr, float* out, int ldo, float* pre_out, int ldp, float* dcolsum, int M, int N, int K,
                            int act, const vh_dropout_spec* drop, void* workspace, size_t workspace_bytes, void* stream) {
    GemmArgs a{};
// ... 93 lines not shown
extern "C" size_t vh_head_greedy_ws_bytes(int B, int V) {
    if (B <= 0 || V <= 0) return 0;
    return HEAD_WS_COUNTERS * sizeof(int) + (size_t)B * ((V + 15) / 16) * sizeof(uint64_t);
}

extern "C" int vh_head_greedy(const float* x, int ldx, const float* proj_w, float* logits, int ldl, int V, int eos,
                              int64_t* codes, int64_t codes_stride, int32_t* eos_count, const int32_t* pos_base,
                              const float* audio_emb, const float* pe, int32_t* audio_pos, int32_t* cache_len, float* x_next,
                              int B, int d, void* workspace, size_t workspace_bytes, void* stream) {
    VH_REQUIRE(x && proj_w && logits && codes && eos_count && audio_emb && pe && audio_pos && cache_len && x_next && workspace,
               VH_EINVAL, "vh_head_greedy: null pointer");
    VH_REQUIRE(B > 0 && V > 0 && ldl >= V && ldx >= d && ldx % 4 == 0, VH_EINVAL,
               "vh_head_greedy: bad dims B=%d V=%d ldl=%d d=%d ldx=%d", B, V, ldl, d, ldx);
    VH_REQUIRE(B <= 64 && (d == 128 || d == 256 || d == 512 || d == 1024), VH_EUNSUPPORTED,
               "vh_head_greedy: B <= 64 rows and d_model in {128, 256, 512, 1024} (B=%d d=%d); use vh_linear + vh_greedy_step",
               B, d);
    VH_REQUIRE(vh_aligned16(x) && vh_aligned16(proj_w) && vh_aligned16(audio_emb) && vh_aligned16(pe) && vh_aligned16(x_next) &&
                   vh_aligned16(workspace),
               VH_EALIGN, "vh_head_greedy: x/proj_w/audio_emb/pe/x_next and the workspace must be 16-byte aligned");
    VH_REQUIRE(workspace_bytes >= vh_head_greedy_ws_bytes(B, V), VH_EINVAL, "vh_head_greedy: workspace of %zu bytes, %zu needed",
               workspace_bytes, vh_head_greedy_ws_bytes(B, V));
    GemmArgs a{};
    a.A = x; a.lda = ldx; a.W = proj_w; a.out = logits; a.ldo = ldl; a.M = B; a.N = V; a.K = d; a.act = VH_ACT_NONE; a.k_len = d;
    dim3 grid((V + 15) / 16);
    if (B > 16) {
        a.rg_rows = ((int)grid.x * ((B + 7) / 8) <= 256) ? 8 : 16;
        grid.z = (B + a.rg_rows - 1) / a.rg_rows;
    }
    HeadStep hs{};
    hs.counters = (int*)workspace;
    hs.cand = (uint64_t*)((char*)workspace + HEAD_WS_COUNTERS * sizeof(int));
    hs.V = V; hs.eos = eos; hs.codes = codes; hs.codes_stride = codes_stride; hs.eos_count = eos_count; hs.pos_base = pos_base;
    hs.audio_emb = audio_emb; hs.pe = pe; hs.audio_pos = audio_pos; hs.cache_len = cache_len; hs.x_next = x_next; hs.d = d;
    hipStream_t s = (hipStream_t)stream;
    if (d % 512 == 0) hipLaunchKernelGGL(gemm_head_greedy_kernel<4>, grid, dim3(512), 0, s, SKINNY_ARGS(a), a, hs);
    else if (d == 256) hipLaunchKernelGGL(gemm_head_greedy_kernel<2>, grid, dim3(512), 0, s, SKINNY_ARGS(a), a, hs);
    else hipLaunchKernelGGL(gemm_head_greedy_kernel<1>, grid, dim3(512), 0, s, SKINNY_ARGS(a), a, hs);
    VH_CHECK_LAUNCH("vh_head_greedy");
    return VH_OK;
}

extern "C" int vh_linear_folded(const float* A, int lda, const float* Wf, const float* c1, const float* c2,
                                const float* residual, int ldr, float* out, int ldo, int M, int N, int K,
                                int act, float ln_eps, void* stream) {
    GemmArgs a{};
    a.A = A; a.lda = lda; a.W = Wf; a.res = residual; a.ldr = ldr; a.out = out;
    a.ldo = ldo; a.M = M; a.N = N; a.K = K; a.act = act; a.k_len = K;
    LnFuse ln{nullptr, nullptr, nullptr, nullptr, ln_eps, c1, c2};
    VH_REQUIRE(act == VH_ACT_NONE || act == VH_ACT_GELU_ERF, VH_EINVAL, "vh_linear_folded: act=%d", act);
    VH_REQUIRE(ldo >= N && (!residual || ldr >= N), VH_EINVAL, "vh_linear_folded: ldo/ldr < N");
    if (int rc = check_gemm("vh_linear_folded", a, ln)) return rc;
    if (int rc = check_folded("vh_linear_folded", a, ln)) return rc;
    return launch_gemm<EPI_PLAIN>("vh_linear_folded", a, ln, (hipStream_t)stream);
}

extern "C" int vh_linear_qkv_folded(const float* A, int lda, const float* Wf, const float* c1, const float* c2,
                                    float* q_out, int ldq, float* kcache, float* vcache,
                                    const int32_t* cache_len, int B, int T, int d_model, int n_heads,
                                    int S_max, float ln_eps, void* stream) {
    VH_REQUIRE(kcache && vcache, VH_EINVAL, "vh_linear_qkv_folded: null cache");
    VH_REQUIRE(B >= 0 && T >= 0 && n_heads > 0 && d_model == n_heads * VH_HEAD_DIM, VH_EUNSUPPORTED,
               "vh_linear_qkv_folded: d_model=%d must equal n_heads=%d x %d", d_model, n_heads, VH_HEAD_DIM);
    VH_REQUIRE(S_max >= T && ldq >= d_model, VH_EINVAL, "vh_linear_qkv_folded: S_max=%d < T=%d or ldq", S_max, T);
    VH_REQUIRE(vh_aligned16(kcache) && vh_aligned16(vcache), VH_EALIGN, "vh_linear_qkv_folded: cache alignment");
    GemmArgs a{};
    a.A = A; a.lda = lda; a.W = Wf; a.out = q_out; a.ldo = ldq;
// ... 106 lines not shown
                            const float* residual, int ldr, float* out, int ldo, int M, int N, int K,
                            int act, void* workspace, size_t workspace_bytes, void* stream) {
    const int splits = splitk_plan(M, N, K);
    if (!splits && workspace && M > 64 && vh_linear_ex_ws_bytes(M, N, K))
        return vh_linear_ex(A, lda, W, bias, residual, ldr, out, ldo, nullptr, 0, nullptr, M, N, K, act, nullptr, workspace,
                            workspace_bytes, stream);
    if (!splits || !workspace)
        return vh_linear(A, lda, W, bias, residual, ldr, out, ldo, M, N, K, act, nullptr, nullptr,
                         nullptr, nullptr, 0.f, stream);
    VH_REQUIRE(workspace_bytes >= vh_linear_ws_bytes(M, N, K) && vh_aligned16(workspace), VH_EINVAL,
               "vh_linear_ws: workspace too small or unaligned (%zu < %zu)", workspace_bytes,
               vh_linear_ws_bytes(M, N, K));
    VH_REQUIRE(act == VH_ACT_NONE || act == VH_ACT_GELU_ERF, VH_EINVAL, "vh_linear_ws: act=%d", act);
    VH_REQUIRE(ldo >= N && (!residual || ldr >= N), VH_EINVAL, "vh_linear_ws: ldo/ldr < N");
    if (M == 0) return VH_OK;
    const int lds_ = (N + 3) / 4 * 4;
    GemmArgs part{};
    float* slabs = (float*)workspace;
    part.A = A; part.lda = lda; part.W = W; part.out = slabs; part.ldo = lds_; part.M = M;
    part.N = N; part.K = K; part.act = VH_ACT_NONE; part.k_len = K / splits;
    LnFuse none{nullptr, nullptr, nullptr, nullptr, 0.f};
    if (int rc = check_gemm("vh_linear_ws", part, none)) return rc;
    GemmArgs fin{};
    fin.bias = bias; fin.res = residual; fin.ldr = ldr; fin.out = out; fin.ldo = ldo; fin.M = M; fin.N = N;
    fin.K = K; fin.act = act;
    VH_REQUIRE(vh_aligned16(out) && vh_aligned16(bias) && vh_aligned16(residual) && ldo % 4 == 0 &&
                   (!residual || ldr % 4 == 0),
               VH_EALIGN, "vh_linear_ws: out/bias/residual alignment");
    hipStream_t s = (hipStream_t)stream;
    if (M > 64) {
        const int tm = (M + TM - 1) / TM, tn = (N + TN - 1) / TN;
        if (part.k_len % TK == 0 && vh_tuning(VH_TUNE_TILE_DMA) != 1)
            hipLaunchKernelGGL((gemm_tile_dma_kernel<EPI_PARTIAL>), dim3(tm * tn, splits), dim3(256), 0, s, part, tm, tn,
                               TailSplit{tm * tn, 1, part.k_len, nullptr});
        else
            hipLaunchKernelGGL((gemm_tile_kernel<EPI_PARTIAL>), dim3(tm * tn, splits), dim3(256), 0, s, part, tm, tn);
        const int items_t = M * (lds_ / 4);
        const int rbt = 256;
        hipLaunchKernelGGL(splitk_reduce_kernel, dim3((items_t + rbt - 1) / rbt), dim3(rbt), 0, s,
                           (const float*)slabs, splits, fin, lds_);
        VH_CHECK_LAUNCH("vh_linear_ws");
        return VH_OK;
    }
    dim3 grid((N + 15) / 16, splits);
    const int mt = (M + 15) / 16;
    if (mt == 1) hipLaunchKernelGGL((gemm_skinny_fast<1, 4, EPI_PARTIAL, 4, 0, 1>), grid, dim3(256), 0, s, SKINNY_ARGS(part), part, none);
    else if (mt == 2) hipLaunchKernelGGL((gemm_skinny_fast<2, 4, EPI_PARTIAL, 4, 0, 1>), grid, dim3(256), 0, s, SKINNY_ARGS(part), part, none);
    else hipLaunchKernelGGL((gemm_skinny_fast<4, 4, EPI_PARTIAL, 4, 0, 1>), grid, dim3(256), 0, s, SKINNY_ARGS(part), part, none);
    const int items = M * (lds_ / 4);
    const int rb = vh_tuning(VH_TUNE_REDUCE_BLOCK) > 0 ? vh_tuning(VH_TUNE_REDUCE_BLOCK) : 128;
    hipLaunchKernelGGL(splitk_reduce_kernel, dim3((items + rb - 1) / rb), dim3(rb), 0, s,
                       (const float*)slabs, splits, fin, lds_);
    VH_CHECK_LAUNCH("vh_linear_ws");
    return VH_OK;
}

#define TN_OPSZ 4224

struct TnArgs {
    const float* A; int lda;
    const float* B; int ldb;
    int M, NI, NJ;
    int m_chunk;
};

__global__ __launch_bounds__(256, 2) void gemm_tile_tn_kernel(TnArgs g, GemmArgs a, int tiles_i, int tiles_j) {
    __shared__ __attribute__((aligned(16))) float lds[2][2][TN_OPSZ];
// ... 294 lines not shown
```

### valle2_amd/csrc/plan.hip

```cpp
#include <stdarg.h>

#include <vector>

#include "vh_common.h"

static thread_local char g_err[512] = "";

void vh_set_error(const char* fmt, ...) {
    va_list ap;
    va_start(ap, fmt);
    vsnprintf(g_err, sizeof(g_err), fmt, ap);
    va_end(ap);
}

static int g_tuning[VH_TUNE_COUNT] = {0};
extern "C" int vh_h16_format(void) { return VH_H16_IS_BF16; }
int vh_tuning(int knob) { return (knob >= 0 && knob < VH_TUNE_COUNT) ? g_tuning[knob] : 0; }
extern "C" int vh_set_tuning(int knob, int value) {
    VH_REQUIRE(knob >= 0 && knob < VH_TUNE_COUNT, VH_EINVAL, "vh_set_tuning: knob=%d", knob);
    g_tuning[knob] = value;
    return VH_OK;
}

extern "C" const char* vh_last_error(void) { return g_err; }
extern "C" int vh_version(void) { return VH_VERSION; }

#define HIP_TRY(call)                                                             \
    do {                                                                          \
        hipError_t e_ = (call);                                                   \
        VH_REQUIRE(e_ == hipSuccess, VH_ELAUNCH, #call ": %s", hipGetErrorString(e_)); \
    } while (0)

#define TRY(call)                \
    do {                         \
        int rc_ = (call);        \
        if (rc_ != VH_OK) return rc_; \
    } while (0)

struct vh_ar_decoder {
    vh_ar_decoder_desc d;
    std::vector<vh_layer> layers;
    hipGraph_t graph = nullptr;
    hipGraphExec_t exec = nullptr;
    hipGraph_t graph_n = nullptr;
    hipGraphExec_t exec_n = nullptr;
    int ldl = 0;
};

static int decoder_check(const vh_ar_decoder_desc* d) {
    VH_REQUIRE(d, VH_EINVAL, "vh_ar_decoder: null desc");
    VH_REQUIRE(d->B > 0 && d->B <= 64, VH_EUNSUPPORTED,
               "vh_ar_decoder: B=%d (decode rows per GPU must be 1..64)", d->B);
    VH_REQUIRE(d->n_layers > 0 && d->layers, VH_EINVAL, "vh_ar_decoder: no layers");
    VH_REQUIRE(d->n_heads > 0 && d->d_model > 0 && d->d_model % d->n_heads == 0, VH_EUNSUPPORTED,
               "vh_ar_decoder: d_model=%d is not a multiple of n_heads=%d", d->d_model, d->n_heads);
    const int hd = d->d_model / d->n_heads;
    if (hd != VH_HEAD_DIM) {
        VH_REQUIRE(hd % 4 == 0 && hd >= 16 && hd <= 256, VH_EUNSUPPORTED,
                   "vh_ar_decoder: head width %d (d_model=%d / n_heads=%d): the cached decoder serves 64 and multiples of 4 "
                   "from 16 to 256", hd, d->d_model, d->n_heads);
        VH_REQUIRE(d->d_model % 16 == 0 && d->d_model <= 1024, VH_EUNSUPPORTED,
                   "vh_ar_decoder: head width %d needs d_model %% 16 == 0 and d_model <= 1024 (got %d)", hd, d->d_model);
        VH_REQUIRE(!d->kv_bf16, VH_EUNSUPPORTED, "vh_ar_decoder: the bf16 K/V cache (perf mode) is width 64 only (head width %d)",
                   hd);
        VH_REQUIRE(d->prefix_len == 0, VH_EUNSUPPORTED,
                   "vh_ar_decoder: the shared prompt (prefix_len=%d) is width 64 only (head width %d)", d->prefix_len, hd);
        VH_REQUIRE(d->n_groups == 0, VH_EUNSUPPORTED,
                   "vh_ar_decoder: grouped shared prompts (n_groups=%d) are width 64 only (head width %d)", d->n_groups, hd);
        VH_REQUIRE(d->n_split == 1 ||
                       (d->attn_partial && d->attn_partial_bytes >= vh_attn_decode_hd_ws_bytes(d->B, d->n_heads, hd, d->n_split)),
                   VH_EINVAL, "vh_ar_decoder: head width %d with n_split=%d needs attn_partial of vh_attn_decode_hd_ws_bytes() = %zu "
                   "bytes (got %zu)", hd, d->n_split, vh_attn_decode_hd_ws_bytes(d->B, d->n_heads, hd, d->n_split),
                   d->attn_partial_bytes);
    } else {
        VH_REQUIRE(d->d_model <= 4096, VH_EUNSUPPORTED, "vh_ar_decoder: d_model=%d: the cached decoder serves d_model <= 4096",
                   d->d_model);
    }
    VH_REQUIRE(d->dff % 16 == 0 && d->V > 0 && d->S_max > 0 && d->n_split >= 1, VH_EINVAL,
               "vh_ar_decoder: bad dff/V/S_max/n_split");
// ... 66 lines not shown
        VH_REQUIRE(!d->head_ws, VH_EUNSUPPORTED,
                   "vh_ar_decoder: row_sampling with head_ws: per-row sampling runs the sampler on every row, head_ws (head + "
                   "greedy step in one launch) has none — set one or the other");
        VH_REQUIRE(vh_aligned16(d->row_sampling), VH_EALIGN, "vh_ar_decoder: row_sampling must be 16-byte aligned");
    }
    if (d->head_ws) {
        VH_REQUIRE(d->top_k == 1 && d->B <= 64 && d->d_model <= 1024, VH_EUNSUPPORTED,
                   "vh_ar_decoder: head_ws (head + greedy step in one launch) is for top_k == 1, B <= 64, d_model <= 1024");
        VH_REQUIRE(d->head_ws_bytes >= vh_head_greedy_ws_bytes(d->B, d->V) && vh_aligned16(d->head_ws), VH_EINVAL,
                   "vh_ar_decoder: head_ws needs vh_head_greedy_ws_bytes() = %zu bytes, 16-byte aligned (got %zu)",
                   vh_head_greedy_ws_bytes(d->B, d->V), d->head_ws_bytes);
    }
    return VH_OK;
}

extern "C" void vh_ar_decoder_destroy(vh_ar_decoder* dec);

extern "C" vh_ar_decoder* vh_ar_decoder_create(const vh_ar_decoder_desc* desc) {
    if (decoder_check(desc) != VH_OK) return nullptr;
    auto* dec = new vh_ar_decoder();
    dec->d = *desc;
    dec->layers.assign(desc->layers, desc->layers + desc->n_layers);
    dec->d.layers = dec->layers.data();
    dec->ldl = (desc->V + 3) & ~3;
    return dec;
}

extern "C" void vh_ar_decoder_destroy(vh_ar_decoder* dec) {
    if (!dec) return;
    if (dec->exec) (void)hipGraphExecDestroy(dec->exec);
    if (dec->graph) (void)hipGraphDestroy(dec->graph);
    if (dec->exec_n) (void)hipGraphExecDestroy(dec->exec_n);
    if (dec->graph_n) (void)hipGraphDestroy(dec->graph_n);
    delete dec;
}

void vh_internal_attn_decode_events(hipEvent_t start, hipEvent_t stop);
void vh_internal_attn_decode_hd_events(hipEvent_t start, hipEvent_t stop);
int vh_internal_linear_w16(const float* A, int lda, const uint16_t* W16, const float* bias, const float* residual, int ldr,
                           float* out, int ldo, int M, int N, int K, void* stream);
int vh_internal_linear_qkv_folded_kv16_w16(const float* A, int lda, const uint16_t* Wf16, const float* c1, const float* c2,
                                           float* q_out, int ldq, uint16_t* kcache16, uint16_t* vcache16, const int32_t* cache_len,
                                           int B, int d_model, int n_heads, int S_max, float ln_eps, void* stream);
int vh_internal_ffn_decode_w16(const float* x, int ldx, const uint16_t* w1f16, const float* c1, const float* c2,
                               const uint16_t* w2_16, const float* b2, float* out, int ldo, int M, int d_model, int dff,
                               float ln_eps, void* workspace, size_t workspace_bytes, void* stream);
int vh_internal_sample_step(const float* logits, int ldl, int V, int eos, int top_k, float top_p, float temperature, uint64_t seed,
                            const uint64_t* seed_dev, const vh_row_sampling* rs, int64_t* codes, int64_t codes_stride, int32_t* eos_count,
                            const int32_t* pos_base, float* sum_logprobs, const float* audio_emb, const float* pe,
                            int32_t* audio_pos, int32_t* cache_len, float* x_next, int B, int d, void* stream);
int vh_internal_sample_step_wide(const float* logits, int ldl, int V, int eos, int top_k, float top_p, float temperature,
                                 uint64_t seed, const uint64_t* seed_dev, const vh_row_sampling* rs, int64_t* codes,
                                 int64_t codes_stride, int32_t* eos_count, const int32_t* pos_base, float* sum_logprobs, const float* audio_emb,
                                 const float* pe, int32_t* audio_pos, int32_t* cache_len, float* x_next, int B, int d,
                                 void* stream);

static int decoder_enqueue(vh_ar_decoder* dec, hipStream_t s, std::vector<hipEvent_t>* ev,
                           std::vector<hipEvent_t>* kev = nullptr) {
    const vh_ar_decoder_desc& d = dec->d;
    const int B = d.B, D = d.d_model;
    const int hd = D / d.n_heads;
    const int ffn_knob = vh_tuning(VH_TUNE_FFN_FUSED);
    const bool ffn_fused = d.ffn_ws && ffn_knob != 1 && (d.d_model <= 512 || d.d_model == 640 || d.d_model == 768 || d.d_model == 896 ||
                                                        (ffn_knob == 2 && d.d_model <= 1024));
    const bool ln_apart = D > 1024;
    auto attention = [&](const vh_layer& L) -> int {
// ... 70 lines not shown
                              d.S_max, nullptr, nullptr, nullptr, nullptr, 0.f, s));
        } else
            TRY(vh_linear_qkv(d.x, D, L.wqkv, d.q, D, L.kcache, L.vcache, d.cache_len, B, 1, D, d.n_heads,
                              d.S_max, L.ln1_g, L.ln1_b, nullptr, nullptr, d.ln_eps, s));
        TRY(run_attention(L));
        if (w16)
            TRY(vh_internal_linear_w16(d.attn, D, L.wo16, L.bo, d.x, D, d.x, D, B, D, D, s));
        else
            TRY(vh_linear(d.attn, D, L.wo, L.bo, d.x, D, d.x, D, B, D, D, VH_ACT_NONE, nullptr, nullptr,
                          nullptr, nullptr, 0.f, s));
        if (w16 && d.ffn_ws) {
            TRY(vh_internal_ffn_decode_w16(d.x, D, L.w1_f16, L.w1_c1, L.w1_c2, L.w2_16, L.b2, d.x, D, B, D, d.dff, d.ln_eps, d.ffn_ws,
                                           d.ffn_ws_bytes, s));
            continue;
        }
        if (ffn_fused) {
            TRY(vh_ffn_decode(d.x, D, L.w1_f, L.w1_c1, L.w1_c2, L.w2, L.b2, d.x, D, B, D, d.dff, d.ln_eps, d.ffn_ws,
                              d.ffn_ws_bytes, s));
            continue;
        }
        if (L.w1_f)
            TRY(vh_linear_folded(d.x, D, L.w1_f, L.w1_c1, L.w1_c2, nullptr, 0, d.hidden, d.dff, B, d.dff, D,
                                 VH_ACT_GELU_ERF, d.ln_eps, s));
        else if (ln_apart) {
            TRY(vh_layernorm(d.x, L.ln2_g, L.ln2_b, nullptr, nullptr, d.attn, B, D, d.ln_eps, s));
            TRY(vh_linear(d.attn, D, L.w1, L.b1, nullptr, 0, d.hidden, d.dff, B, d.dff, D, VH_ACT_GELU_ERF,
                          nullptr, nullptr, nullptr, nullptr, 0.f, s));
        } else
            TRY(vh_linear(d.x, D, L.w1, L.b1, nullptr, 0, d.hidden, d.dff, B, d.dff, D, VH_ACT_GELU_ERF,
                          L.ln2_g, L.ln2_b, nullptr, nullptr, d.ln_eps, s));
        TRY(vh_linear_ws(d.hidden, d.dff, L.w2, L.b2, d.x, D, d.x, D, B, D, d.dff, VH_ACT_NONE, d.gemm_ws,
                         d.gemm_ws_bytes, s));
    }
    if (d.top_k == 1 && d.head_ws) {
        TRY(vh_head_greedy(d.x, D, d.proj_w, d.logits, dec->ldl, d.V, d.eos, d.codes, d.codes_stride, d.eos_count, d.pos_base,
                           d.audio_emb, d.audio_pe, d.audio_pos, d.cache_len, d.x, B, D, d.head_ws, d.head_ws_bytes, s));
        return VH_OK;
    }
    if (d.kv_bf16 && d.proj_w16 && D <= 1024)
        TRY(vh_internal_linear_w16(d.x, D, d.proj_w16, nullptr, nullptr, 0, d.logits, dec->ldl, B, d.V, D, s));
    else
        TRY(vh_linear(d.x, D, d.proj_w, nullptr, nullptr, 0, d.logits, dec->ldl, B, d.V, D, VH_ACT_NONE,
                      nullptr, nullptr, nullptr, nullptr, 0.f, s));
    if (d.top_k == 1 && !d.row_sampling)
        TRY(vh_greedy_step(d.logits, dec->ldl, d.V, d.eos, d.codes, d.codes_stride, d.eos_count,
                           d.pos_base, d.audio_emb, d.audio_pe, d.audio_pos, d.cache_len, d.x, B, D, s));
    else if (d.V > 2048)
        TRY(vh_internal_sample_step_wide(d.logits, dec->ldl, d.V, d.eos, d.top_k, d.top_p, d.temperature, d.seed, d.seed_dev,
                                         d.row_sampling, d.codes, d.codes_stride, d.eos_count, d.pos_base, d.sum_logprobs, d.audio_emb,
                                         d.audio_pe, d.audio_pos, d.cache_len, d.x, B, D, s));
    else
        TRY(vh_internal_sample_step(d.logits, dec->ldl, d.V, d.eos, d.top_k, d.top_p, d.temperature, d.seed, d.seed_dev,
                                    d.row_sampling, d.codes, d.codes_stride, d.eos_count, d.pos_base, d.sum_logprobs, d.audio_emb,
                                    d.audio_pe, d.audio_pos, d.cache_len, d.x, B, D, s));
    return VH_OK;
}

extern "C" int vh_ar_decoder_step(vh_ar_decoder* dec, void* stream) {
    VH_REQUIRE(dec, VH_EINVAL, "vh_ar_decoder_step: null decoder");
    return decoder_enqueue(dec, (hipStream_t)stream, nullptr);
}

#define VH_GRAPH_STEPS 8

static int capture_steps(vh_ar_decoder* dec, hipStream_t s, int n_steps, hipGraph_t* graph, hipGraphExec_t* exec) {
    if (*exec) { (void)hipGraphExecDestroy(*exec); *exec = nullptr; }
    if (*graph) { (void)hipGraphDestroy(*graph); *graph = nullptr; }
    hipError_t e = hipStreamBeginCapture(s, hipStreamCaptureModeThreadLocal);
    VH_REQUIRE(e == hipSuccess, VH_ELAUNCH, "hipStreamBeginCapture: %s", hipGetErrorString(e));
    int rc = VH_OK;
    for (int i = 0; i < n_steps && rc == VH_OK; ++i) rc = decoder_enqueue(dec, s, nullptr);
    e = hipStreamEndCapture(s, graph);
    if (rc != VH_OK) return rc;
    VH_REQUIRE(e == hipSuccess && *graph, VH_ELAUNCH, "hipStreamEndCapture: %s", hipGetErrorString(e));
    e = hipGraphInstantiate(exec, *graph, nullptr, nullptr, 0);
    VH_REQUIRE(e == hipSuccess, VH_ELAUNCH, "hipGraphInstantiate: %s", hipGetErrorString(e));
    return VH_OK;
}

extern "C" int vh_ar_decoder_capture(vh_ar_decoder* dec, void* stream) {
    VH_REQUIRE(dec, VH_EINVAL, "vh_ar_decoder_capture: null decoder");
    VH_REQUIRE(stream, VH_EINVAL, "vh_ar_decoder_capture: capture needs a non-null stream");
    hipStream_t s = (hipStream_t)stream;
    TRY(capture_steps(dec, s, 1, &dec->graph, &dec->exec));
    if (vh_tuning(VH_TUNE_GRAPH_STEPS) != 1) TRY(capture_steps(dec, s, VH_GRAPH_STEPS, &dec->graph_n, &dec->exec_n));
    return VH_OK;
}

extern "C" int vh_ar_decoder_replay(vh_ar_decoder* dec, int n_steps, void* stream) {
    VH_REQUIRE(dec && dec->exec, VH_ESTATE, "vh_ar_decoder_replay: capture first");
    VH_REQUIRE(n_steps >= 0, VH_EINVAL, "vh_ar_decoder_replay: n_steps=%d", n_steps);
    hipStream_t s = (hipStream_t)stream;
    int i = 0;
    if (dec->exec_n)
        for (; i + VH_GRAPH_STEPS <= n_steps; i += VH_GRAPH_STEPS) HIP_TRY(hipGraphLaunch(dec->exec_n, s));
    for (; i < n_steps; ++i) HIP_TRY(hipGraphLaunch(dec->exec, s));
    return VH_OK;
}

static float mean_event_pairs(std::vector<hipEvent_t>& ev) {
    double total = 0.0;
    int n = 0;
    for (size_t i = 0; i + 1 < ev.size(); i += 2) {
        float ms = 0.f;
        if (hipEventElapsedTime(&ms, ev[i], ev[i + 1]) == hipSuccess) { total += ms; ++n; }
    }
    for (hipEvent_t e : ev) (void)hipEventDestroy(e);
    ev.clear();
    return n ? (float)(total / n) : 0.f;
}

extern "C" int vh_ar_decoder_profile_attn(vh_ar_decoder* dec, int n_steps, void* stream,
                                          float* mean_ms, float* floor_ms, float* kernel_ms) {
    VH_REQUIRE(dec && mean_ms && n_steps > 0, VH_EINVAL, "vh_ar_decoder_profile_attn: bad args");
    hipStream_t s = (hipStream_t)stream;
    std::vector<hipEvent_t> ev, fl, kev;
    int rc = VH_OK;
    for (int i = 0; i < n_steps && rc == VH_OK; ++i) {
        rc = decoder_enqueue(dec, s, &ev, kernel_ms ? &kev : nullptr);
        hipEvent_t f0, f1;
        if (floor_ms && hipEventCreate(&f0) == hipSuccess && hipEventCreate(&f1) == hipSuccess) {
            (void)hipEventRecord(f0, s);
            (void)hipEventRecord(f1, s);
            fl.push_back(f0);
            fl.push_back(f1);
        }
    }
    (void)hipStreamSynchronize(s);
    if (floor_ms) *floor_ms = mean_event_pairs(fl);
    if (kernel_ms) *kernel_ms = mean_event_pairs(kev);
    *mean_ms = mean_event_pairs(ev);
    return rc;
}

extern "C" int vh_transformer_forward(const vh_forward_desc* f, void* stream) {
    VH_REQUIRE(f && f->layers && f->x && f->xn && f->q && f->attn && f->hidden, VH_EINVAL,
               "vh_transformer_forward: null pointer in desc");
    VH_REQUIRE(f->B > 0 && f->T > 0 && f->n_layers > 0 && f->S_max >= f->T, VH_EINVAL,
               "vh_transformer_forward: bad dims B=%d T=%d L=%d S_max=%d", f->B, f->T, f->n_layers,
               f->S_max);
    VH_REQUIRE(f->d_model == f->n_heads * VH_HEAD_DIM, VH_EUNSUPPORTED,
               "vh_transformer_forward: d_model=%d != n_heads=%d x 64", f->d_model, f->n_heads);
    const int B = f->B, T = f->T, D = f->d_model, M = B * T;
    for (int i = 0; i < f->n_layers; ++i) {
        const vh_layer& L = f->layers[i];
        const float* ada = f->ada ? f->ada + (int64_t)i * 4 * D : nullptr;
        const float* src = (i == 0 && f->x_in) ? f->x_in : f->x;
        TRY(vh_layernorm(src, L.ln1_g, L.ln1_b, ada, ada ? ada + D : nullptr, f->xn, M, D, f->ln_eps,
                         stream));
        TRY(vh_linear_qkv(f->xn, D, L.wqkv, f->q, D, L.kcache, L.vcache, nullptr, B, T, D, f->n_heads,
                          f->S_max, nullptr, nullptr, nullptr, nullptr, 0.f, stream));
        TRY(vh_attn_rows(f->q, D, L.kcache, L.vcache, f->attn, D, B, f->n_heads, T, T, f->S_max,
                         f->mode, f->x_len, f->x_len_dev, f->kv_len, f->mask, f->pad, stream));
        TRY(vh_linear_ws(f->attn, D, L.wo, L.bo, src, D, f->x, D, M, D, D, VH_ACT_NONE, f->gemm_ws,
                         f->gemm_ws_bytes, stream));
        TRY(vh_layernorm(f->x, L.ln2_g, L.ln2_b, ada ? ada + 2 * D : nullptr, ada ? ada + 3 * D : nullptr,
                         f->xn, M, D, f->ln_eps, stream));
        TRY(vh_linear_ws(f->xn, D, L.w1, L.b1, nullptr, 0, f->hidden, f->dff, M, f->dff, D, VH_ACT_GELU_ERF,
                         f->gemm_ws, f->gemm_ws_bytes, stream));
        TRY(vh_linear_ws(f->hidden, f->dff, L.w2, L.b2, f->x, D, f->x, D, M, D, f->dff, VH_ACT_NONE, f->gemm_ws,
                         f->gemm_ws_bytes, stream));
    }
    return VH_OK;
}
```

### valle2_amd/csrc/vh_common.h

```cpp
#pragma once
#include <hip/hip_runtime.h>
#include <stdint.h>
#include <stdio.h>

#include "../../include/valle_hip.h"

typedef float f32x4 __attribute__((ext_vector_type(4)));
typedef float f32x16 __attribute__((ext_vector_type(16)));

#ifdef VH_PERF_BF16
#define VH_H16_IS_BF16 1
typedef __bf16 vh_h16;
#else
#define VH_H16_IS_BF16 0
typedef _Float16 vh_h16;
#endif
typedef vh_h16 vh_h16x2 __attribute__((ext_vector_type(2)));
typedef vh_h16 vh_h16x8 __attribute__((ext_vector_type(8)));
__device__ __forceinline__ uint32_t vh_pack_h16(float lo, float hi) {
#if VH_H16_IS_BF16
    const vh_h16x2 r = {(__bf16)lo, (__bf16)hi};
#else
    const vh_h16x2 r = {(_Float16)lo, (_Float16)hi};
#endif
// ... 23 lines not shown
#if VH_H16_IS_BF16
#define VH_MFMA16(a, b, c) __builtin_amdgcn_mfma_f32_32x32x16_bf16(a, b, c, 0, 0, 0)
#else
#define VH_MFMA16(a, b, c) __builtin_amdgcn_mfma_f32_32x32x16_f16(a, b, c, 0, 0, 0)
#endif

#define VH_Q16_PRESCALE 0.18033688011112042f

#define VH_WAVE 64

void vh_set_error(const char* fmt, ...);

#define VH_REQUIRE(cond, code, ...)      \
    do {                                 \
        if (!(cond)) {                   \
            vh_set_error(__VA_ARGS__);   \
            return (code);               \
        }                                \
    } while (0)

static inline bool vh_aligned16(const void* p) { return (reinterpret_cast<uintptr_t>(p) & 15u) == 0; }

#define VH_CHECK_LAUNCH(name)                                                      \
    do {                                                                           \
        hipError_t e_ = hipGetLastError();                                         \
        if (e_ != hipSuccess) {                                                    \
            vh_set_error("%s: launch failed: %s", name, hipGetErrorString(e_));    \
            return VH_ELAUNCH;                                                     \
        }                                                                          \
    } while (0)

int vh_tuning(int knob);

template <int CTRL, int ROW_MASK>
__device__ __forceinline__ float dpp_get(float v, float identity) {
    return __int_as_float(__builtin_amdgcn_update_dpp(__float_as_int(identity), __float_as_int(v), CTRL,
                                                      ROW_MASK, 0xF, false));
}
__device__ __forceinline__ float row16_sum(float v) {
    v += dpp_get<0xB1, 0xF>(v, 0.f);
    v += dpp_get<0x4E, 0xF>(v, 0.f);
    v += dpp_get<0x141, 0xF>(v, 0.f);
    v += dpp_get<0x140, 0xF>(v, 0.f);
    return v;
}
__device__ __forceinline__ float row16_max(float v) {
    v = fmaxf(v, dpp_get<0xB1, 0xF>(v, v));
    v = fmaxf(v, dpp_get<0x4E, 0xF>(v, v));
    v = fmaxf(v, dpp_get<0x141, 0xF>(v, v));
    v = fmaxf(v, dpp_get<0x140, 0xF>(v, v));
    return v;
}
__device__ __forceinline__ float rows4_sum(float v) {
    v += dpp_get<0x142, 0xA>(v, 0.f);
    v += dpp_get<0x143, 0xC>(v, 0.f);
    return __int_as_float(__builtin_amdgcn_readlane(__float_as_int(v), 63));
}
__device__ __forceinline__ float rows4_max(float v) {
    v = fmaxf(v, dpp_get<0x142, 0xA>(v, v));
    v = fmaxf(v, dpp_get<0x143, 0xC>(v, v));
    return __int_as_float(__builtin_amdgcn_readlane(__float_as_int(v), 63));
}
__device__ __forceinline__ float wave_sum(float v) { return rows4_sum(row16_sum(v)); }
__device__ __forceinline__ float wave_max(float v) { return rows4_max(row16_max(v)); }
__device__ __forceinline__ f32x4 ld4(const float* p) { return *reinterpret_cast<const f32x4*>(p); }
__device__ __forceinline__ f32x4 ld4_stream(const float* p) {
    return __builtin_nontemporal_load(reinterpret_cast<const f32x4*>(p));
}
__device__ __forceinline__ void st4(float* p, f32x4 v) { *reinterpret_cast<f32x4*>(p) = v; }

__device__ __forceinline__ float vh_exp2(float x) { return __builtin_amdgcn_exp2f(x); }

__device__ __forceinline__ float vh_erf(float x) {
    const float s = x * x;
    float p = -5.654105917e-04f;
    p = fmaf(p, s, 4.923277535e-03f);
    p = fmaf(p, s, -2.671638504e-02f);
    p = fmaf(p, s, 1.128036454e-01f);
    p = fmaf(p, s, -3.761234879e-01f);
    p = fmaf(p, s, 1.128379107e+00f);
    const float small = p * x;
    const float t = fminf(fabsf(x), 4.0f);
    float q = -1.920139221e-05f;
    q = fmaf(q, t, 4.581596004e-04f);
    q = fmaf(q, t, -4.958351608e-03f);
    q = fmaf(q, t, 3.263662755e-02f);
    q = fmaf(q, t, -1.490577757e-01f);
    q = fmaf(q, t, 5.206782818e-01f);
    q = fmaf(q, t, -1.624367833e+00f);
    q = fmaf(q, t, -1.092074905e-03f);
    q = fmaf(-1.4426950408889634f * t, t, q);
    const float large = copysignf(1.0f - __builtin_amdgcn_exp2f(q), x);
    return fabsf(x) < 1.0f ? small : large;
}

typedef float vh_f32x2 __attribute__((ext_vector_type(2)));
__device__ __forceinline__ vh_f32x2 vh_splat2(float v) { return vh_f32x2{v, v}; }
__device__ __forceinline__ vh_f32x2 gelu_erf2(vh_f32x2 x) {
    const vh_f32x2 z = x * vh_splat2(0.70710678118654752440f);
    const vh_f32x2 s = z * z;
    vh_f32x2 p = vh_splat2(-5.654105917e-04f);
    p = __builtin_elementwise_fma(p, s, vh_splat2(4.923277535e-03f));
// ... 104 lines not shown
```

### valle2_amd/engine.py

```python
from __future__ import annotations

import ctypes as C
import os
import threading
import weakref

import torch

from . import _lib, kernels
from ._lib import VhArDecoderDesc, VhForwardDesc, VhLayer, check, ptr, stream

HEAD_DIM = kernels.HEAD_DIM


class KVCache:

    def __init__(self, n_layers, batch, n_heads, s_max, device, dtype=torch.float32, head_dim=HEAD_DIM):
        self.buf = torch.empty(n_layers, 2, batch, n_heads, s_max, head_dim, device=device, dtype=dtype)
        self.n_layers, self.batch, self.n_heads, self.s_max = n_layers, batch, n_heads, s_max
        self.head_dim = head_dim

    @property
    def bf16(self):
        return self.buf.dtype == kernels.H16
# ... 240 lines not shown
        ada = adaln_table(transformer, embedding)
    desc = _lib.VhForward16Desc(
        B=B, T=T, d_model=d, n_heads=cfg.n_heads, dff=cfg.dim_feedforward, n_layers=cfg.num_layers, S_max=cache.s_max,
        mode=mode, x_len=int(x_len), ln_eps=1e-5, layers=table, layers16=t16, ada=ptr(ada), x_len_dev=ptr(x_len_dev),
        kv_len=ptr(kv_len), x=ptr(x), x_in=ptr(x_in), xn16=scratch.xn.data_ptr(), q16=scratch.q.data_ptr(),
        attn16=scratch.attn.data_ptr(), hidden16=scratch.hidden.data_ptr())
    check(_lib.lib().vh_transformer_forward_bf16(C.byref(desc), stream()), 'vh_transformer_forward_bf16')
    return x


class ForwardScratch:
    def __init__(self, rows, d, dff, device):
        self.xn = torch.empty(rows, d, device=device, dtype=torch.float32)
        self.q = torch.empty(rows, d, device=device, dtype=torch.float32)
        self.attn = torch.empty(rows, d, device=device, dtype=torch.float32)
        self.hidden = torch.empty(rows, dff, device=device, dtype=torch.float32)
        L = _lib.lib()
        self.ws_bytes = max(L.vh_linear_ws_bytes(rows, d, d), L.vh_linear_ws_bytes(rows, d, dff),
                            L.vh_linear_ws_bytes(rows, dff, d))
        self.ws = torch.zeros(self.ws_bytes // 4, device=device, dtype=torch.float32) if self.ws_bytes else None
        self.d, self.dff = d, dff

    def fit(self, rows):
        L = _lib.lib()
        need = max(L.vh_linear_ws_bytes(rows, self.d, self.d), L.vh_linear_ws_bytes(rows, self.d, self.dff),
                   L.vh_linear_ws_bytes(rows, self.dff, self.d))
        if need > self.ws_bytes:
            self.ws_bytes = need
            self.ws = torch.zeros(need // 4, device=self.xn.device, dtype=torch.float32)
        return self


def transformer_forward(transformer, x, cache: KVCache, *, mode, x_len=0, x_len_dev=None,
                        kv_len=None, mask=None, pad=None, embedding=None, scratch=None, x_in=None):
    cfg = transformer.hparams
    B, T, d = x.shape
    if not x.is_contiguous():
        raise _lib.VhError('x must be contiguous')
    if x_in is not None and (tuple(x_in.shape) != tuple(x.shape) or x_in.dtype != torch.float32):
        raise _lib.VhError('x_in must match x')
    if d != cfg.n_heads * HEAD_DIM:
        kv = cache if cache is not None and getattr(cache, 'head_dim', HEAD_DIM) == d // cfg.n_heads else None
        return _transformer_forward_generic(transformer, x, mode=mode, x_len=x_len, x_len_dev=x_len_dev, kv_len=kv_len,
                                            mask=mask, pad=pad, embedding=embedding, x_in=x_in, cache=kv)
    if cache is None or cache.batch != B or cache.s_max < T or cache.n_layers != cfg.num_layers:
        raise _lib.VhError('KV cache does not fit this forward')
    scratch = scratch or ForwardScratch(B * T, d, cfg.dim_feedforward, x.device)
    table = layer_table(transformer, cache)
    ada = None
    if cfg.norm != 'LayerNorm':
        if embedding is None:
            raise TypeError('AdaptiveLayerNorm needs `embedding` (reference: Linear(None) TypeError)')
        ada = adaln_table(transformer, embedding)
    desc = VhForwardDesc(
        B=B, T=T, d_model=d, n_heads=cfg.n_heads, dff=cfg.dim_feedforward, n_layers=cfg.num_layers,
        S_max=cache.s_max, mode=mode, x_len=int(x_len), ln_eps=1e-5, layers=table, ada=ptr(ada),
        x_len_dev=ptr(x_len_dev), kv_len=ptr(kv_len), mask=ptr(mask), pad=ptr(pad),
        x=ptr(x), xn=ptr(scratch.xn), q=ptr(scratch.q), attn=ptr(scratch.attn),
        hidden=ptr(scratch.hidden), gemm_ws=ptr(scratch.ws), gemm_ws_bytes=scratch.ws_bytes, x_in=ptr(x_in))
    check(_lib.lib().vh_transformer_forward(C.byref(desc), stream()), 'vh_transformer_forward')
    return x


def _transformer_forward_generic(transformer, x, *, mode, x_len, x_len_dev, kv_len, mask, pad, embedding, x_in, cache=None):
    cfg = transformer.hparams
    B, T, d = x.shape
    h = cfg.n_heads
    hd = d // h
    if hd % 4:
        raise _lib.VhError(f'head_dim {hd}: the general attention path needs a multiple of 4')
    if cache is not None and (cache.bf16 or cache.head_dim != hd or cache.batch != B or cache.s_max < T
                              or cache.n_layers != cfg.num_layers or cache.n_heads != h):
        raise _lib.VhError('KV cache does not fit this forward')
    ada = None
    if cfg.norm != 'LayerNorm':
        if embedding is None:
            raise TypeError('AdaptiveLayerNorm needs `embedding` (reference: Linear(None) TypeError)')
        ada = adaln_table(transformer, embedding)
    cur = (x_in if x_in is not None else x).reshape(B * T, d)
    spec = dict(mode=mode, x_len=int(x_len), x_len_dev=x_len_dev, kv_len=kv_len, mask=mask, pad=pad)
    f32 = dict(device=x.device, dtype=torch.float32)
    for i, layer in enumerate(transformer.layers):
        g1, b1, wqkv, wo, bo, g2, b2, w1, bb1, w2, bb2 = (t.detach() for t in _layer_params(layer))
        sc1, sh1, sc2, sh2 = (ada[i, 0, 0], ada[i, 0, 1], ada[i, 1, 0], ada[i, 1, 1]) if ada is not None else (None,) * 4
        xn = kernels.layernorm(cur, g1, b1, ada_scale=sc1, ada_shift=sh1, eps=layer.norm1.eps)
        qkv = kernels.linear(xn, wqkv, out=torch.empty(B * T, 3 * d, **f32))
        if cache is not None:
            kernels.kv_store(qkv, cache.k(i), cache.v(i), B, T)
        q, k, v = (qkv.view(B, T, 3, h, hd)[:, :, j].permute(0, 2, 1, 3) for j in range(3))
        attn = torch.empty(B * T, d, **f32)
        kernels.attn_generic(q, k, v, attn.view(B, T, h, hd).permute(0, 2, 1, 3), hd ** -0.5, **spec)
        nxt = kernels.linear(attn, wo, bo, residual=cur, out=torch.empty(B * T, d, **f32))
        xn = kernels.layernorm(nxt, g2, b2, ada_scale=sc2, ada_shift=sh2, eps=layer.norm2.eps)
        hid = kernels.linear(xn, w1, bb1, act=kernels.ACT_GELU, out=torch.empty(B * T, w1.shape[0], **f32))
# ... 260 lines not shown
            audio_pos=ptr(audio_pos), eos_count=ptr(self.eos_count), pos_base=ptr(pos_base),
            codes=ptr(codes), codes_stride=codes.stride(0), top_k=self.sampling[0], top_p=self.sampling[1],
            temperature=self.sampling[2], seed=0 if self.seed_dev is not None else self.sampling[3] & (2 ** 64 - 1),
            seed_dev=ptr(self.seed_dev), proj_w16=ptr(self._proj16),
            sum_logprobs=ptr(self.sum_logprobs), ffn_ws=ptr(self.ffn_ws), ffn_ws_bytes=ffn_bytes,
            kv_bf16=int(self.kv_bf16), prefix_len=self.prefix_len if prefix is not None else 0,
            prefix_S=prefix.s_max if prefix is not None else 0,
            n_groups=prefix.batch if self.grouped else 0, beams_per_group=self.beams if self.grouped else 0,
            prefix_cap=self.prefix_cap if self.grouped else 0, prefix_lens=ptr(prefix_lens) if self.grouped else None,
            attn_partial_bytes=self.partial.numel() * 4 if self.partial is not None else 0,
            head_ws=ptr(self.head_ws), head_ws_bytes=self.head_ws.numel() * 4 if self.head_ws is not None else 0,
            row_sampling=ptr(self.row_sampling))
        self._desc = desc
        self._h = _lib.lib().vh_ar_decoder_create(C.byref(desc))
        if not self._h:
            msg = _lib.lib().vh_last_error()
            raise _lib.VhError(f'vh_ar_decoder_create: {msg.decode() if msg else "failed"}')
        self._captured = False
        self.use_graph = use_graph

    def close(self):
        if getattr(self, '_h', None) and _lib is not None:
            _lib.lib().vh_ar_decoder_destroy(self._h)
            self._h = None

    __del__ = close

    def reset(self, seed=0):
        self.eos_count.zero_()
        self.sum_logprobs.zero_()
        self.sampling = self.sampling[:3] + (int(seed),)
        if self.seed_dev is not None:
            self.seed_dev.copy_(torch.tensor([int(seed)], dtype=torch.int64), non_blocking=True)

    def capture(self):
        if self.use_graph and not self._captured:
            with _CAPTURE_LOCK:
                cap = _capture_stream(torch.cuda.current_device())
                check(_lib.lib().vh_ar_decoder_capture(self._h, cap.cuda_stream), 'vh_ar_decoder_capture')
            self._captured = True

    def run(self, n_steps):
        if n_steps <= 0:
            return
        s = stream()
        L = _lib.lib()
        if self.use_graph:
            self.capture()
            check(L.vh_ar_decoder_replay(self._h, n_steps, s), 'vh_ar_decoder_replay')
        else:
            for _ in range(n_steps):
                check(L.vh_ar_decoder_step(self._h, s), 'vh_ar_decoder_step')

    def profile_attn(self, n_steps):
        ms, floor, kern = C.c_float(0), C.c_float(0), C.c_float(0)
        check(_lib.lib().vh_ar_decoder_profile_attn(self._h, n_steps, stream(), C.byref(ms), C.byref(floor),
                                                    C.byref(kern)), 'vh_ar_decoder_profile_attn')
        return ms.value, floor.value, kern.value
```

### valle2_amd/generation.py

```python
from __future__ import annotations

import os
import threading
import time
from dataclasses import dataclass

import torch

from . import _lib, kernels
from . import sampling as _sampling
from .engine import (MAX_DECODE_D_MODEL, ArDecoder, ForwardScratch, ForwardScratch16, KVCache, QueueSchedule, StepSampler,
                     cached_decode_supported, ffn_fused_width, group_prefix_cap, grouped_prompts_fit, perf_forward_supported,
                     queue_steps_cap, transformer_forward, transformer_forward_bf16)
from .utils import get_best_beam

EOS_POLL = 32
MAX_DECODE_ROWS = 64
SHARED_PROMPT = os.environ.get('VALLE2_SHARED_PROMPT', '1') != '0'
_DECODER_ENV = ('VALLE2_HEAD_FUSED', 'VALLE2_SHARED_SPLIT', 'VALLE2_FOLD_LN', 'VALLE2_DECODE_W16')
DECODER_SLOTS = int(os.environ.get('VALLE2_DECODER_SLOTS', '2'))
_SLOT_LOCK = threading.Lock()

RECOMPUTE_GENERAL = 'RECOMPUTE_GENERAL'
ROWS_HD = 'ROWS_HD'
SHARED = 'SHARED'
GROUPED = 'GROUPED'
ROWS_PERF_PREFILL = 'ROWS_PERF_PREFILL'
ROWS = 'ROWS'


def roundup32(n):
    return (n + 31) // 32 * 32


def _check_int(entry, name, value):
    if not isinstance(value, int) or isinstance(value, bool) or value < 1:
        raise ValueError(f'{entry}: {name}={value!r} (an integer >= 1)')


def _check_grouped_decoder(entry, cfg, beams, needs):
    if not cfg.use_kv_cache or cfg.d_model != cfg.n_heads * kernels.HEAD_DIM or cfg.d_model > MAX_DECODE_D_MODEL:
        raise ValueError(f'{entry}: beams={beams} with use_kv_cache={cfg.use_kv_cache}, d_model={cfg.d_model}, '
                         f'n_heads={cfg.n_heads}: {needs} the cached decoder at head width '
                         f'{kernels.HEAD_DIM} (d_model <= {MAX_DECODE_D_MODEL})')


def check_sampling(sampling, n, forced=None):
    sampling = _sampling.check_list('generate_batch', sampling, n)
    if sampling is not None and forced is not None:
# ... 243 lines not shown
        assert prompt_tokens.dim() == 1, 'Prompt tokens should be 1D tensor.'
        assert prompt_codes.dim() == 2, 'Prompt codes should be 2D tensor.'
        if target_tokens is not None:
            assert target_tokens.dim() == 1, 'Target tokens should be 1D tensor.'
        texts.append(prompt_tokens if target_tokens is None else torch.cat((prompt_tokens, target_tokens), dim=0))
        firsts.append(prompt_codes[..., 0])
    return texts, firsts


def best_beam_tokens(model, rows, sum_logprobs, prompt_len):
    best = get_best_beam(rows, sum_logprobs, model.eos_token, model.config.length_penalty)[prompt_len:]
    return best[best != model.eos_token]


def prompt_pass(model, plan, state, texts, first_codes):
    cfg, dev, d = model.config, model.device, model.config.d_model
    B, s0, n, codes = plan.B, plan.s0, plan.beams, state.codes
    i32 = dict(device=dev, dtype=torch.int32)
    rows = 1 if plan.kind == SHARED else plan.G
    text_ids = None
    if not plan.ragged:
        text_ids = torch.stack(texts[:rows])
        codes[:, 1:plan.pl_max] = torch.stack(first_codes).repeat_interleave(n, 0) if plan.kind == GROUPED else torch.stack(first_codes)
        x = torch.empty(rows, s0, d, device=dev, dtype=torch.float32)
        model._embed_rows(text_ids, codes[:rows * n:n, :plan.pl_max], x)
        fwd = dict(x_len=plan.txs[0])
    else:
        x = torch.zeros(plan.G, s0, d, device=dev, dtype=torch.float32)
        for b in range(plan.G):
            codes[b * n:(b + 1) * n, 1:plan.pls[b]] = first_codes[b]
            model._embed_rows(texts[b].unsqueeze(0), codes[b * n:b * n + 1, :plan.pls[b]], x[b:b + 1])
        fwd = dict(x_len_dev=torch.tensor(plan.txs, **i32), kv_len=torch.tensor(plan.ctx, **i32))
    into = state.cache if state.prefix is None else state.prefix
    if plan.prefill_bf16:
        transformer_forward_bf16(model.transformer, x, into, mode=kernels.MASK_PREFIX,
                                 scratch=ForwardScratch16(rows * s0, d, cfg.dim_feedforward, dev), **fwd)
    elif plan.kind == SHARED and plan.perf_mode:
        wide = KVCache(cfg.num_layers, 1, cfg.n_heads, state.prefix.s_max, dev)
        transformer_forward(model.transformer, x, wide, mode=kernels.MASK_PREFIX,
                            scratch=ForwardScratch(s0, d, cfg.dim_feedforward, dev), **fwd)
        wide.narrow_into(state.prefix)
    else:
        scratch = None if plan.kind in (RECOMPUTE_GENERAL, ROWS_HD) else ForwardScratch(rows * s0, d, cfg.dim_feedforward, dev)
        transformer_forward(model.transformer, x, into, mode=kernels.MASK_PREFIX, scratch=scratch, **fwd)
    if plan.ragged:
        last = x[torch.arange(plan.G, device=dev), fwd['kv_len'].long() - 1]
    elif plan.kind == SHARED:
        last = x[:, -1].expand(B, d)
    else:
        last = x[:, -1]
    if plan.kind == GROUPED:
        last = last.repeat_interleave(n, 0)
    if plan.kind == ROWS and plan.perf_mode:
        state.cache = state.cache.narrowed(plan.s_max)
    return last.contiguous(), fwd, text_ids


def _decode_forced(model, plan, dec, forced, keep_logits):
    dev, d = model.device, model.config.d_model
    forced = forced.to(dev)
    if plan.ragged or forced.numel() < plan.max_new:
        raise ValueError('forced: one token per step, equal-length rows')
    pe, kept = model.audio_position_emb.pe, {}
    for t in range(plan.max_new):
        if t:
            dec.run(1)
        if t in keep_logits:
            kept[t] = dec.logits[:, : dec.V].clone()
        dec.codes[:, plan.pl_max + t] = forced[t]
        kernels.embed_sum_pe(dec.codes[:, plan.pl_max + t:plan.pl_max + t + 1], [model.audio_emb.weight.detach()], pe,
                             plan.pl_max + t, dec.x.view(plan.B, 1, d))
    return kept


def _decode_recompute(model, plan, dec, texts, cache, fwd, text_ids):
    cfg, dev, d = model.config, model.device, model.config.d_model
    B, s0, codes = plan.B, plan.s0, dec.codes
    scratch = None if plan.kind == RECOMPUTE_GENERAL else ForwardScratch(B * (s0 + plan.max_new), d, cfg.dim_feedforward, dev)
    rows_idx = torch.arange(B, device=dev)
    done = 1
    while done < plan.max_new:
        t = done
        xs = (torch.zeros if plan.ragged else torch.empty)(B, s0 + t, d, device=dev, dtype=torch.float32)
        if scratch is not None:
            scratch.fit(B * (s0 + t))
        if not plan.ragged:
            model._embed_rows(text_ids, codes[:, :plan.pl_max + t], xs)
            transformer_forward(model.transformer, xs, cache, mode=kernels.MASK_PREFIX, scratch=scratch, **fwd)
            last = xs[:, -1]
        else:
            for b in range(B):
                model._embed_rows(texts[b].unsqueeze(0), codes[b:b + 1, :plan.pls[b] + t], xs[b:b + 1])
            transformer_forward(model.transformer, xs, cache, mode=kernels.MASK_PREFIX, scratch=scratch,
                                x_len_dev=fwd['x_len_dev'], kv_len=fwd['kv_len'] + t)
            last = xs[rows_idx, fwd['kv_len'].long() + t - 1]
        dec.sample_from(last.contiguous())
        done += 1
        if done % EOS_POLL == 0 and bool((dec.eos_count[:done] == B).any()):
            break
    return done


def _decode_cached(plan, dec, done):
    while done < plan.max_new:
        n = min(EOS_POLL, plan.max_new - done)
        dec.run(n)
        done += n
        full = (dec.eos_count[:done] == plan.B).nonzero()
        if full.numel():
            return done, int(full[0])
    return done, None


def _generate_in_groups(model, texts, first_codes, max_new, use_graph, perf_mode, beams=1, sampling=None):
    B, dev = len(texts) * beams, model.device
    parts, stats = [], []
    per = MAX_DECODE_ROWS // beams
    for r0 in range(0, len(texts), per):
        parts.append(model.generate_batch(texts[r0:r0 + per], first_codes[r0:r0 + per],
                                          max_new=max_new, use_graph=use_graph, perf_mode=perf_mode, beams=beams,
                                          sampling=None if sampling is None else sampling[r0:r0 + per]))
        stats.append(model.last_generate_stats)
    width = max(p.shape[1] for p in parts)
    out = torch.full((B, width), model.eos_token, device=dev, dtype=torch.int64)
    r = 0
    for p in parts:
        out[r:r + p.shape[0], :p.shape[1]] = p
        r += p.shape[0]
    merged = dict(stats[-1])
    merged['prompt_lens'] = [x for st in stats for x in st['prompt_lens']]
    merged['sum_logprobs'] = torch.cat([st['sum_logprobs'] for st in stats])
    merged['tokens_appended'] = max(st['tokens_appended'] for st in stats)
    merged['groups'] = sum(st['groups'] for st in stats)
    model.last_generate_stats = merged
    return out

# ... 219 lines not shown
```

Baseline: 49130 tokens/s.

## Compute only last prompt rows in final prefill layer and run decode until EOS on device

```diff
diff --git a/include/valle_hip.h b/include/valle_hip.h
--- a/include/valle_hip.h
+++ b/include/valle_hip.h
@@ -8,7 +8,7 @@
 extern "C" {
 #endif
 
-#define VH_VERSION 135
+#define VH_VERSION 136
 #define VH_MAX_TABLES 32
 #define VH_SAMPLE_MAX_V 16384
 #define VH_HEAD_DIM 64
@@ -46,7 +46,9 @@
        VH_TUNE_ATTN_BWD = 13,
        VH_TUNE_ATTN_BWD_CHUNKS = 14,
        VH_TUNE_BF16_GEMM = 15,
-       VH_TUNE_COUNT = 16 };
+       VH_TUNE_EOS_RUN = 16,
+       VH_TUNE_PROMPT_TAIL = 17,
+       VH_TUNE_COUNT = 18 };
 int vh_set_tuning(int knob, int value);
 
 typedef struct { uint64_t seed; uint64_t site; float p; } vh_dropout_spec;
@@ -263,6 +265,9 @@
 int vh_ar_decoder_step(vh_ar_decoder* dec, void* stream);
 int vh_ar_decoder_capture(vh_ar_decoder* dec, void* stream);
 int vh_ar_decoder_replay(vh_ar_decoder* dec, int n_steps, void* stream);
+int vh_ar_decoder_run(vh_ar_decoder* dec, int max_steps, void* stream, int* steps_run, int* stop_step);
+int vh_ar_decoder_rearm(vh_ar_decoder* dec);
+int vh_ar_decoder_word_scope(vh_ar_decoder* dec, int on);
 int vh_ar_decoder_profile_attn(vh_ar_decoder* dec, int n_steps, void* stream, float* mean_ms,
                                float* floor_ms, float* kernel_ms);
 
@@ -325,6 +330,8 @@
     void *gemm_ws;
     size_t gemm_ws_bytes;
     const float *x_in;
+    const int32_t *last_rows;
+    float *last_out;
 } vh_forward_desc;
 int vh_transformer_forward(const vh_forward_desc* desc, void* stream);
 
diff --git a/valle2_amd/_lib.py b/valle2_amd/_lib.py
--- a/valle2_amd/_lib.py
+++ b/valle2_amd/_lib.py
@@ -68,6 +68,7 @@
         ('x_len_dev', C.c_void_p), ('kv_len', C.c_void_p), ('mask', C.c_void_p), ('pad', C.c_void_p),
         ('x', C.c_void_p), ('xn', C.c_void_p), ('q', C.c_void_p), ('attn', C.c_void_p),
         ('hidden', C.c_void_p), ('gemm_ws', C.c_void_p), ('gemm_ws_bytes', C.c_size_t), ('x_in', C.c_void_p),
+        ('last_rows', C.c_void_p), ('last_out', C.c_void_p),
     ]
 
 
@@ -193,6 +194,9 @@
     'vh_ar_decoder_step': (C.c_int, [C.c_void_p, C.c_void_p]),
     'vh_ar_decoder_capture': (C.c_int, [C.c_void_p, C.c_void_p]),
     'vh_ar_decoder_replay': (C.c_int, [C.c_void_p, C.c_int, C.c_void_p]),
+    'vh_ar_decoder_run': (C.c_int, [C.c_void_p, C.c_int, C.c_void_p, C.POINTER(C.c_int), C.POINTER(C.c_int)]),
+    'vh_ar_decoder_rearm': (C.c_int, [C.c_void_p]),
+    'vh_ar_decoder_word_scope': (C.c_int, [C.c_void_p, C.c_int]),
     'vh_ar_decoder_profile_attn': (C.c_int, [C.c_void_p, C.c_int, C.c_void_p,
                                              C.POINTER(C.c_float), C.POINTER(C.c_float), C.POINTER(C.c_float)]),
     'vh_layernorm_bwd': (C.c_int, [c_f32p, c_f32p, c_f32p, c_f32p, c_f32p, c_f32p, c_f32p, c_f32p, c_f32p,
@@ -251,12 +255,18 @@
     def set_tuning(knob, value):
         global TUNING_EPOCH
         TUNING_EPOCH += 1
-        return raw_set(knob, value)
+        rc = raw_set(knob, value)
+        if rc == 0:
+            TUNING[knob] = value
+        return rc
     lib.vh_set_tuning = set_tuning
     return lib
 
 
 TUNING_EPOCH = 0
+TUNING = {}
+TUNE_EOS_RUN = 16
+TUNE_PROMPT_TAIL = 17
 
 
 def h16_dtype():
diff --git a/valle2_amd/csrc/attention.hip b/valle2_amd/csrc/attention.hip
--- a/valle2_amd/csrc/attention.hip
+++ b/valle2_amd/csrc/attention.hip
@@ -521,15 +521,17 @@
     int n_qblocks;
     float* lse2;
     int64_t mask_bstride;
+    const int32_t* last_rows;
 };
 
-__global__ __launch_bounds__(256, 2) void attn_rows_kernel(RowsArgs a) {
-    __shared__ __attribute__((aligned(16))) float lds[2 * 2 * KT * KLD];
+template <bool ONLY>
+__device__ __forceinline__ void attn_rows_body(const RowsArgs& a, float* lds) {
     const int tid = threadIdx.x, lane = tid & 63, w = tid >> 6;
     const int r = lane & 31, h = lane >> 5;
-    const int n_bh = gridDim.x / a.n_qblocks;
+    const int n_bh = ONLY ? gridDim.x : gridDim.x / a.n_qblocks;
     const int bh = blockIdx.x % n_bh, b = bh / a.n_heads, head = bh - b * a.n_heads;
-    const int q0 = (a.n_qblocks - 1 - (int)(blockIdx.x / n_bh)) * QB;
+    const int q0 = ONLY ? (min(max(a.last_rows[b], 0), a.Tq - 1) / QB) * QB
+                        : (a.n_qblocks - 1 - (int)(blockIdx.x / n_bh)) * QB;
     const int q_off = a.Tk - a.Tq;
     const int kvl = a.kv_len ? min(a.kv_len[b], a.Tk) : a.Tk;
     const int xl = a.x_len_dev ? a.x_len_dev[b] : a.x_len;
@@ -680,10 +682,21 @@
     }
 }
 
+__global__ __launch_bounds__(256, 2) void attn_rows_kernel(RowsArgs a) {
+    __shared__ __attribute__((aligned(16))) float lds[2 * 2 * KT * KLD];
+    attn_rows_body<false>(a, lds);
+}
+
+__global__ __launch_bounds__(256, 2) void attn_rows_last_kernel(RowsArgs a) {
+    __shared__ __attribute__((aligned(16))) float lds[2 * 2 * KT * KLD];
+    attn_rows_body<true>(a, lds);
+}
+
 static int attn_rows_launch(const float* q, int ldq, const float* kcache, const float* vcache,
                             float* out, int ldo, int B, int n_heads, int Tq, int Tk, int S_max,
                             int mode, int x_len, const int32_t* x_len_dev, const int32_t* kv_len,
-                            const uint8_t* mask, const uint8_t* pad, float* lse2, void* stream, int64_t mask_bstride = 0) {
+                            const uint8_t* mask, const uint8_t* pad, float* lse2, void* stream, int64_t mask_bstride = 0,
+                            const int32_t* last_rows = nullptr) {
     VH_REQUIRE(q && kcache && vcache && out, VH_EINVAL, "vh_attn_rows: null pointer");
     VH_REQUIRE(B >= 0 && n_heads > 0 && Tq >= 0 && Tk >= Tq && S_max >= Tk, VH_EINVAL,
                "vh_attn_rows: bad dims B=%d h=%d Tq=%d Tk=%d S_max=%d", B, n_heads, Tq, Tk, S_max);
@@ -697,11 +710,22 @@
     if (B == 0 || Tq == 0) return VH_OK;
     const int nqb = (Tq + QB - 1) / QB;
     RowsArgs a{q, ldq, kcache, vcache, out, ldo, n_heads, Tq, Tk, S_max, mode, x_len,
-               x_len_dev, kv_len, mask, pad, nqb, lse2, mask_bstride};
-    dim3 grid(nqb * B * n_heads);
-    hipLaunchKernelGGL(attn_rows_kernel, grid, dim3(256), 0, (hipStream_t)stream, a);
+               x_len_dev, kv_len, mask, pad, nqb, lse2, mask_bstride, last_rows};
+    if (last_rows)
+        hipLaunchKernelGGL(attn_rows_last_kernel, dim3(B * n_heads), dim3(256), 0, (hipStream_t)stream, a);
+    else
+        hipLaunchKernelGGL(attn_rows_kernel, dim3(nqb * B * n_heads), dim3(256), 0, (hipStream_t)stream, a);
     VH_CHECK_LAUNCH("vh_attn_rows");
     return VH_OK;
+}
+
+int vh_internal_attn_rows_last(const float* q, int ldq, const float* kcache, const float* vcache, float* out, int ldo, int B,
+                               int n_heads, int Tq, int Tk, int S_max, int mode, int x_len, const int32_t* x_len_dev,
+                               const int32_t* kv_len, const uint8_t* mask, const uint8_t* pad, const int32_t* last_rows,
+                               void* stream) {
+    VH_REQUIRE(last_rows, VH_EINVAL, "vh_attn_rows (last rows): null last_rows");
+    return attn_rows_launch(q, ldq, kcache, vcache, out, ldo, B, n_heads, Tq, Tk, S_max, mode, x_len, x_len_dev, kv_len, mask,
+                            pad, nullptr, stream, 0, last_rows);
 }
 
 extern "C" int vh_attn_rows(const float* q, int ldq, const float* kcache, const float* vcache,
diff --git a/valle2_amd/csrc/elementwise.hip b/valle2_amd/csrc/elementwise.hip
--- a/valle2_amd/csrc/elementwise.hip
+++ b/valle2_amd/csrc/elementwise.hip
@@ -272,11 +272,28 @@
     return VH_OK;
 }
 
+__global__ __launch_bounds__(256) void gather_rows_kernel(const float* __restrict__ x, int T, const int32_t* __restrict__ rows,
+                                                          float* __restrict__ out, int d) {
+    const int b = blockIdx.x;
+    const int r = min(max(rows[b], 0), T - 1);
+    const float* src = x + ((int64_t)b * T + r) * d;
+    for (int c = threadIdx.x * 4; c < d; c += 1024) st4(out + (int64_t)b * d + c, ld4(src + c));
+}
+
+int vh_internal_gather_rows(const float* x, int T, const int32_t* rows, float* out, int B, int d, void* stream) {
+    VH_REQUIRE(x && rows && out && B > 0 && T > 0 && d > 0 && d % 4 == 0, VH_EINVAL, "gather rows: bad arguments B=%d T=%d d=%d", B, T, d);
+    VH_REQUIRE(vh_aligned16(x) && vh_aligned16(out), VH_EALIGN, "gather rows: x / out must be 16-byte aligned");
+    hipLaunchKernelGGL(gather_rows_kernel, dim3(B), dim3(256), 0, (hipStream_t)stream, x, T, rows, out, d);
+    VH_CHECK_LAUNCH("gather rows");
+    return VH_OK;
+}
+
 __global__ __launch_bounds__(256) void greedy_step_kernel(
     const float* __restrict__ logits, int ldl, int V, int eos, int64_t* __restrict__ codes,
     int64_t codes_stride, int32_t* __restrict__ eos_count, const int32_t* __restrict__ pos_base,
     const float* __restrict__ audio_emb, const float* __restrict__ pe,
-    int32_t* __restrict__ audio_pos, int32_t* __restrict__ cache_len, float* __restrict__ x_next, int d) {
+    int32_t* __restrict__ audio_pos, int32_t* __restrict__ cache_len, float* __restrict__ x_next, int d,
+    int32_t* __restrict__ all_eos) {
     __shared__ float s_val[4];
     __shared__ int s_idx[4];
     __shared__ int s_tok;
@@ -305,7 +322,7 @@
         int tok = bi;
         if (row[pos - 1] == (int64_t)eos) tok = eos;
         row[pos] = tok;
-        if (tok == eos) atomicAdd(&eos_count[pos - (pos_base ? pos_base[b] : 0)], 1);
+        if (tok == eos) vh_count_eos(eos_count, pos - (pos_base ? pos_base[b] : 0), gridDim.x, all_eos);
         s_tok = tok;
     }
     __syncthreads();
@@ -334,7 +351,7 @@
                "vh_greedy_step: audio_emb/pe/x_next must be 16-byte aligned");
     hipLaunchKernelGGL(greedy_step_kernel, dim3(B), dim3(256), 0, (hipStream_t)stream, logits, ldl,
                        V, eos, codes, codes_stride, eos_count, pos_base, audio_emb, pe, audio_pos,
-                       cache_len, x_next, d);
+                       cache_len, x_next, d, vh_internal_all_eos_word());
     VH_CHECK_LAUNCH("vh_greedy_step");
     return VH_OK;
 }
@@ -372,7 +389,7 @@
     const int32_t* __restrict__ pos_base, float* __restrict__ sum_logprobs,
     const float* __restrict__ audio_emb, const float* __restrict__ pe, int32_t* __restrict__ audio_pos,
     int32_t* __restrict__ cache_len, float* __restrict__ x_next, int d, int npow2, const uint64_t* __restrict__ seed_dev,
-    const vh_row_sampling* __restrict__ rs) {
+    const vh_row_sampling* __restrict__ rs, int32_t* __restrict__ all_eos) {
     uint32_t draw_key = blockIdx.x;
     bool greedy = false;
     if (rs) {
@@ -557,7 +574,7 @@
         if (sum_logprobs && !finished) sum_logprobs[b] += pick_logprob;
         if (finished) tok = eos;
         row[pos] = tok;
-        if (tok == eos) atomicAdd(&eos_count[pos - (pos_base ? pos_base[b] : 0)], 1);
+        if (tok == eos) vh_count_eos(eos_count, pos - (pos_base ? pos_base[b] : 0), gridDim.x, all_eos);
         s_tok = tok;
     }
     __syncthreads();
@@ -591,7 +608,8 @@
     while (npow2 < V) npow2 <<= 1;
     hipLaunchKernelGGL(sample_step_kernel, dim3(B), dim3(256), 0, (hipStream_t)stream, logits, ldl, V,
                        eos, top_k, top_p, rs ? 1.0f : 1.0f / temperature, seed, codes, codes_stride, eos_count,
-                       pos_base, sum_logprobs, audio_emb, pe, audio_pos, cache_len, x_next, d, npow2, seed_dev, rs);
+                       pos_base, sum_logprobs, audio_emb, pe, audio_pos, cache_len, x_next, d, npow2, seed_dev, rs,
+                       vh_internal_all_eos_word());
     VH_CHECK_LAUNCH("vh_sample_step");
     return VH_OK;
 }
@@ -673,7 +691,7 @@
     const int32_t* __restrict__ pos_base, float* __restrict__ sum_logprobs,
     const float* __restrict__ audio_emb, const float* __restrict__ pe, int32_t* __restrict__ audio_pos,
     int32_t* __restrict__ cache_len, float* __restrict__ x_next, int d, const uint64_t* __restrict__ seed_dev,
-    const vh_row_sampling* __restrict__ rs) {
+    const vh_row_sampling* __restrict__ rs, int32_t* __restrict__ all_eos) {
     uint32_t draw_key = blockIdx.x;
     bool greedy = false;
     if (rs) {
@@ -838,7 +856,7 @@
         if (sum_logprobs && !finished) sum_logprobs[b] += pick_logprob;
         if (finished) tok = eos;
         row[pos] = tok;
-        if (tok == eos) atomicAdd(&eos_count[pos - (pos_base ? pos_base[b] : 0)], 1);
+        if (tok == eos) vh_count_eos(eos_count, pos - (pos_base ? pos_base[b] : 0), gridDim.x, all_eos);
         s_tok = tok;
     }
     __syncthreads();
@@ -870,7 +888,8 @@
                "vh_sample_step_wide: audio_emb/pe/x_next must be 16-byte aligned");
     hipLaunchKernelGGL(sample_step_wide_kernel, dim3(B), dim3(WIDE_THREADS), 0, (hipStream_t)stream, logits, ldl, V,
                        eos, top_k, top_p, rs ? 1.0f : 1.0f / temperature, seed, codes, codes_stride, eos_count,
-                       pos_base, sum_logprobs, audio_emb, pe, audio_pos, cache_len, x_next, d, seed_dev, rs);
+                       pos_base, sum_logprobs, audio_emb, pe, audio_pos, cache_len, x_next, d, seed_dev, rs,
+                       vh_internal_all_eos_word());
     VH_CHECK_LAUNCH("vh_sample_step_wide");
     return VH_OK;
 }
diff --git a/valle2_amd/csrc/gemm.hip b/valle2_amd/csrc/gemm.hip
--- a/valle2_amd/csrc/gemm.hip
+++ b/valle2_amd/csrc/gemm.hip
@@ -59,6 +59,8 @@
     int32_t* cache_len;
     float* x_next;
     int d;
+    int rows;
+    int32_t* all_eos;
 };
 
 __device__ __forceinline__ uint32_t vh_bf16_bits(float x) {
@@ -403,7 +405,7 @@
         pw[i] = a.W + (int64_t)min(n0 + row, a.N - 1) * a.K + skq + blockIdx.y * a.k_len;
     }
     auto gload1 = [&](int i, int k0) {
-        const int kk = k0 + skq < a.k_len ? k0 : 0;
+        const int kk = k0 + skq < a.k_len ? k0 : -skq;
         ra[i] = ld4(pa[i] + kk);
         rw[i] = ld4(pw[i] + kk);
     };
@@ -485,9 +487,11 @@
 struct TailSplit {
     int n_whole, split, k_len;
     float* ws;
+    const int32_t* keep_rows;
+    int keep_T, keep_B;
 };
 
-template <int EPI, bool DROP = false>
+template <int EPI, bool DROP = false, bool KEEP = false>
 __global__ __launch_bounds__(256, 2) void gemm_tile_dma_kernel(GemmArgs a, int tiles_m, int tiles_n, TailSplit ts) {
     __shared__ __attribute__((aligned(16))) float lds[2][2][TM * LDS_LD];
     __builtin_amdgcn_s_setprio(3);
@@ -506,6 +510,17 @@
     const int tile = tail ? nwg + unit / ts.split
                           : (xcd < r8 ? xcd * (q8 + 1) : r8 * (q8 + 1) + (xcd - r8) * q8) + bid / 8;
     const int m0 = (tile / tiles_n) * TM, n0 = (tile % tiles_n) * TN;
+    if constexpr (KEEP) {
+        if (!tail) {
+            bool keep = false;
+            const int b1 = min((m0 + TM - 1) / ts.keep_T, ts.keep_B - 1);
+            for (int b = m0 / ts.keep_T; b <= b1; ++b) {
+                const int row = b * ts.keep_T + ts.keep_rows[b];
+                keep = keep || (row >= m0 && row < m0 + TM);
+            }
+            if (!keep) return;
+        }
+    }
     const int k_len = tail ? ts.k_len : a.k_len;
     const int k_ofs = tail ? (unit % ts.split) * ts.k_len : blockIdx.y * a.k_len;
 
@@ -1081,7 +1096,7 @@
             int tok = min(bi, hs->V - 1);
             if (crow[pos - 1] == (int64_t)hs->eos) tok = hs->eos;
             crow[pos] = tok;
-            if (tok == hs->eos) atomicAdd(&hs->eos_count[pos - (hs->pos_base ? hs->pos_base[b] : 0)], 1);
+            if (tok == hs->eos) vh_count_eos(hs->eos_count, pos - (hs->pos_base ? hs->pos_base[b] : 0), hs->rows, hs->all_eos);
             s_tok[row] = tok;
             s_pos[row] = pos;
             hs->audio_pos[b] = pos + 1;
@@ -1234,6 +1249,10 @@
     if (splits) return (size_t)splits * M * ((N + 3) / 4 * 4) * sizeof(float);
     return M > 64 ? vh_linear_ex_ws_bytes(M, N, K) : 0;
 }
+
+static thread_local const int32_t* g_keep_rows = nullptr;
+static thread_local int g_keep_T = 0, g_keep_B = 0;
+void vh_internal_gemm_keep_rows(const int32_t* rows, int T, int B) { g_keep_rows = rows; g_keep_T = T; g_keep_B = B; }
 
 static int check_gemm(const char* name, const GemmArgs& a, const LnFuse& ln) {
     VH_REQUIRE(a.A && a.W && a.out, VH_EINVAL, "%s: null pointer", name);
@@ -1416,15 +1435,25 @@
         if (a.w16) { vh_set_error("%s: 16-bit weights are the decode step's form (M <= 64)", name); return VH_EUNSUPPORTED; }
         const int tm = (a.M + TM - 1) / TM, tn = (a.N + TN - 1) / TN;
         if (a.k_len % TK == 0 && vh_tuning(VH_TUNE_TILE_DMA) != 1) {
-            TailSplit ts{tm * tn, 1, a.K, nullptr};
+            TailSplit ts{tm * tn, 1, a.K, nullptr, nullptr, 0, 0};
             if constexpr (EPI == EPI_PLAIN) {
                 int n_whole;
                 const int split = tail_ws ? tail_plan(a.M, a.N, a.K, &n_whole) : 0;
                 if (split && tail_ws_bytes >= (size_t)(tm * tn - n_whole) * split * TM * TN * sizeof(float))
-                    ts = TailSplit{n_whole, split, a.K / split, tail_ws};
+                    ts = TailSplit{n_whole, split, a.K / split, tail_ws, nullptr, 0, 0};
             }
             const int tail = tm * tn - ts.n_whole;
-            if (EPI == EPI_PLAIN && a.drop.thresh)
+            bool kept = false;
+            if constexpr (EPI == EPI_PLAIN) {
+                if (g_keep_rows && !a.drop.thresh && g_keep_T > 0 && g_keep_B > 0 && (int64_t)g_keep_T * g_keep_B == a.M) {
+                    ts.keep_rows = g_keep_rows; ts.keep_T = g_keep_T; ts.keep_B = g_keep_B;
+                    hipLaunchKernelGGL((gemm_tile_dma_kernel<EPI_PLAIN, false, true>), dim3(ts.n_whole + tail * ts.split), dim3(256),
+                                       0, s, a, tm, tn, ts);
+                    kept = true;
+                }
+            }
+            if (kept) {
+            } else if (EPI == EPI_PLAIN && a.drop.thresh)
                 hipLaunchKernelGGL((gemm_tile_dma_kernel<EPI, EPI == EPI_PLAIN>), dim3(ts.n_whole + tail * ts.split), dim3(256), 0,
                                    s, a, tm, tn, ts);
             else
@@ -1584,6 +1613,7 @@
     hs.cand = (uint64_t*)((char*)workspace + HEAD_WS_COUNTERS * sizeof(int));
     hs.V = V; hs.eos = eos; hs.codes = codes; hs.codes_stride = codes_stride; hs.eos_count = eos_count; hs.pos_base = pos_base;
     hs.audio_emb = audio_emb; hs.pe = pe; hs.audio_pos = audio_pos; hs.cache_len = cache_len; hs.x_next = x_next; hs.d = d;
+    hs.rows = B; hs.all_eos = vh_internal_all_eos_word();
     hipStream_t s = (hipStream_t)stream;
     if (d % 512 == 0) hipLaunchKernelGGL(gemm_head_greedy_kernel<4>, grid, dim3(512), 0, s, SKINNY_ARGS(a), a, hs);
     else if (d == 256) hipLaunchKernelGGL(gemm_head_greedy_kernel<2>, grid, dim3(512), 0, s, SKINNY_ARGS(a), a, hs);
@@ -1756,7 +1786,7 @@
         const int tm = (M + TM - 1) / TM, tn = (N + TN - 1) / TN;
         if (part.k_len % TK == 0 && vh_tuning(VH_TUNE_TILE_DMA) != 1)
             hipLaunchKernelGGL((gemm_tile_dma_kernel<EPI_PARTIAL>), dim3(tm * tn, splits), dim3(256), 0, s, part, tm, tn,
-                               TailSplit{tm * tn, 1, part.k_len, nullptr});
+                               TailSplit{tm * tn, 1, part.k_len, nullptr, nullptr, 0, 0});
         else
             hipLaunchKernelGGL((gemm_tile_kernel<EPI_PARTIAL>), dim3(tm * tn, splits), dim3(256), 0, s, part, tm, tn);
         const int items_t = M * (lds_ / 4);
diff --git a/valle2_amd/csrc/plan.hip b/valle2_amd/csrc/plan.hip
--- a/valle2_amd/csrc/plan.hip
+++ b/valle2_amd/csrc/plan.hip
@@ -21,6 +21,10 @@
     g_tuning[knob] = value;
     return VH_OK;
 }
+
+static thread_local int32_t* g_all_eos_word = nullptr;
+void vh_internal_set_all_eos_word(int32_t* word) { g_all_eos_word = word; }
+int32_t* vh_internal_all_eos_word(void) { return g_all_eos_word; }
 
 extern "C" const char* vh_last_error(void) { return g_err; }
 extern "C" int vh_version(void) { return VH_VERSION; }
@@ -45,6 +49,9 @@
     hipGraph_t graph_n = nullptr;
     hipGraphExec_t exec_n = nullptr;
     int ldl = 0;
+    volatile int32_t* eos_word = nullptr;
+    int32_t* eos_word_dev = nullptr;
+    hipEvent_t run_ev[2] = {nullptr, nullptr};
 };
 
 static int decoder_check(const vh_ar_decoder_desc* d) {
@@ -177,6 +184,9 @@
     if (dec->graph) (void)hipGraphDestroy(dec->graph);
     if (dec->exec_n) (void)hipGraphExecDestroy(dec->exec_n);
     if (dec->graph_n) (void)hipGraphDestroy(dec->graph_n);
+    for (hipEvent_t e : dec->run_ev)
+        if (e) (void)hipEventDestroy(e);
+    if (dec->eos_word) (void)hipHostFree((void*)dec->eos_word);
     delete dec;
 }
 
@@ -313,6 +323,10 @@
         TRY(vh_linear_ws(d.hidden, d.dff, L.w2, L.b2, d.x, D, d.x, D, B, D, d.dff, VH_ACT_NONE, d.gemm_ws,
                          d.gemm_ws_bytes, s));
     }
+    struct WordScope {
+        explicit WordScope(int32_t* w) { vh_internal_set_all_eos_word(w); }
+        ~WordScope() { vh_internal_set_all_eos_word(nullptr); }
+    } word_scope(dec->eos_word_dev);
     if (d.top_k == 1 && d.head_ws) {
         TRY(vh_head_greedy(d.x, D, d.proj_w, d.logits, dec->ldl, d.V, d.eos, d.codes, d.codes_stride, d.eos_count, d.pos_base,
                            d.audio_emb, d.audio_pe, d.audio_pos, d.cache_len, d.x, B, D, d.head_ws, d.head_ws_bytes, s));
@@ -363,6 +377,14 @@
     VH_REQUIRE(dec, VH_EINVAL, "vh_ar_decoder_capture: null decoder");
     VH_REQUIRE(stream, VH_EINVAL, "vh_ar_decoder_capture: capture needs a non-null stream");
     hipStream_t s = (hipStream_t)stream;
+    if (!dec->eos_word) {
+        void* w = nullptr;
+        HIP_TRY(hipHostMalloc(&w, sizeof(int32_t), hipHostMallocMapped));
+        dec->eos_word = (volatile int32_t*)w;
+        *dec->eos_word = -1;
+        HIP_TRY(hipHostGetDevicePointer((void**)&dec->eos_word_dev, w, 0));
+        for (hipEvent_t& e : dec->run_ev) HIP_TRY(hipEventCreateWithFlags(&e, hipEventDisableTiming));
+    }
     TRY(capture_steps(dec, s, 1, &dec->graph, &dec->exec));
     if (vh_tuning(VH_TUNE_GRAPH_STEPS) != 1) TRY(capture_steps(dec, s, VH_GRAPH_STEPS, &dec->graph_n, &dec->exec_n));
     return VH_OK;
@@ -376,6 +398,37 @@
     if (dec->exec_n)
         for (; i + VH_GRAPH_STEPS <= n_steps; i += VH_GRAPH_STEPS) HIP_TRY(hipGraphLaunch(dec->exec_n, s));
     for (; i < n_steps; ++i) HIP_TRY(hipGraphLaunch(dec->exec, s));
+    return VH_OK;
+}
+
+extern "C" int vh_ar_decoder_rearm(vh_ar_decoder* dec) {
+    VH_REQUIRE(dec, VH_EINVAL, "vh_ar_decoder_rearm: null decoder");
+    if (dec->eos_word) *dec->eos_word = -1;
+    return VH_OK;
+}
+
+extern "C" int vh_ar_decoder_word_scope(vh_ar_decoder* dec, int on) {
+    VH_REQUIRE(dec, VH_EINVAL, "vh_ar_decoder_word_scope: null decoder");
+    vh_internal_set_all_eos_word(on ? dec->eos_word_dev : nullptr);
+    return VH_OK;
+}
+
+extern "C" int vh_ar_decoder_run(vh_ar_decoder* dec, int max_steps, void* stream, int* steps_run, int* stop_step) {
+    VH_REQUIRE(dec && dec->exec && dec->eos_word, VH_ESTATE, "vh_ar_decoder_run: capture first");
+    VH_REQUIRE(max_steps >= 0, VH_EINVAL, "vh_ar_decoder_run: max_steps=%d", max_steps);
+    hipStream_t s = (hipStream_t)stream;
+    int enq = 0, launches = 0;
+    while (enq < max_steps && *dec->eos_word < 0) {
+        const bool bulk = dec->exec_n && enq + VH_GRAPH_STEPS <= max_steps;
+        HIP_TRY(hipGraphLaunch(bulk ? dec->exec_n : dec->exec, s));
+        enq += bulk ? VH_GRAPH_STEPS : 1;
+        HIP_TRY(hipEventRecord(dec->run_ev[launches & 1], s));
+        if (launches) HIP_TRY(hipEventSynchronize(dec->run_ev[(launches - 1) & 1]));
+        ++launches;
+    }
+    if (launches) HIP_TRY(hipEventSynchronize(dec->run_ev[(launches - 1) & 1]));
+    if (steps_run) *steps_run = enq;
+    if (stop_step) *stop_step = *dec->eos_word;
     return VH_OK;
 }
 
@@ -414,6 +467,13 @@
     return rc;
 }
 
+int vh_internal_attn_rows_last(const float* q, int ldq, const float* kcache, const float* vcache, float* out, int ldo, int B,
+                               int n_heads, int Tq, int Tk, int S_max, int mode, int x_len, const int32_t* x_len_dev,
+                               const int32_t* kv_len, const uint8_t* mask, const uint8_t* pad, const int32_t* last_rows,
+                               void* stream);
+void vh_internal_gemm_keep_rows(const int32_t* rows, int T, int B);
+int vh_internal_gather_rows(const float* x, int T, const int32_t* rows, float* out, int B, int d, void* stream);
+
 extern "C" int vh_transformer_forward(const vh_forward_desc* f, void* stream) {
     VH_REQUIRE(f && f->layers && f->x && f->xn && f->q && f->attn && f->hidden, VH_EINVAL,
                "vh_transformer_forward: null pointer in desc");
@@ -423,16 +483,28 @@
     VH_REQUIRE(f->d_model == f->n_heads * VH_HEAD_DIM, VH_EUNSUPPORTED,
                "vh_transformer_forward: d_model=%d != n_heads=%d x 64", f->d_model, f->n_heads);
     const int B = f->B, T = f->T, D = f->d_model, M = B * T;
+    VH_REQUIRE(!f->last_rows == !f->last_out, VH_EINVAL, "vh_transformer_forward: last_rows and last_out go together");
+    const bool trim = f->last_rows && vh_tuning(VH_TUNE_PROMPT_TAIL) != 1;
+    struct KeepScope {
+        explicit KeepScope(const int32_t* rows, int T, int B) { vh_internal_gemm_keep_rows(rows, T, B); }
+        ~KeepScope() { vh_internal_gemm_keep_rows(nullptr, 0, 0); }
+    };
     for (int i = 0; i < f->n_layers; ++i) {
         const vh_layer& L = f->layers[i];
+        const bool tail_only = trim && i == f->n_layers - 1;
         const float* ada = f->ada ? f->ada + (int64_t)i * 4 * D : nullptr;
         const float* src = (i == 0 && f->x_in) ? f->x_in : f->x;
         TRY(vh_layernorm(src, L.ln1_g, L.ln1_b, ada, ada ? ada + D : nullptr, f->xn, M, D, f->ln_eps,
                          stream));
         TRY(vh_linear_qkv(f->xn, D, L.wqkv, f->q, D, L.kcache, L.vcache, nullptr, B, T, D, f->n_heads,
                           f->S_max, nullptr, nullptr, nullptr, nullptr, 0.f, stream));
-        TRY(vh_attn_rows(f->q, D, L.kcache, L.vcache, f->attn, D, B, f->n_heads, T, T, f->S_max,
-                         f->mode, f->x_len, f->x_len_dev, f->kv_len, f->mask, f->pad, stream));
+        if (tail_only)
+            TRY(vh_internal_attn_rows_last(f->q, D, L.kcache, L.vcache, f->attn, D, B, f->n_heads, T, T, f->S_max, f->mode,
+                                           f->x_len, f->x_len_dev, f->kv_len, f->mask, f->pad, f->last_rows, stream));
+        else
+            TRY(vh_attn_rows(f->q, D, L.kcache, L.vcache, f->attn, D, B, f->n_heads, T, T, f->S_max,
+                             f->mode, f->x_len, f->x_len_dev, f->kv_len, f->mask, f->pad, stream));
+        KeepScope keep(tail_only ? f->last_rows : nullptr, T, B);
         TRY(vh_linear_ws(f->attn, D, L.wo, L.bo, src, D, f->x, D, M, D, D, VH_ACT_NONE, f->gemm_ws,
                          f->gemm_ws_bytes, stream));
         TRY(vh_layernorm(f->x, L.ln2_g, L.ln2_b, ada ? ada + 2 * D : nullptr, ada ? ada + 3 * D : nullptr,
@@ -442,5 +514,6 @@
         TRY(vh_linear_ws(f->hidden, f->dff, L.w2, L.b2, f->x, D, f->x, D, M, D, f->dff, VH_ACT_NONE, f->gemm_ws,
                          f->gemm_ws_bytes, stream));
     }
-    return VH_OK;
-}
+    if (f->last_rows) TRY(vh_internal_gather_rows(f->x, T, f->last_rows, f->last_out, B, D, stream));
+    return VH_OK;
+}
diff --git a/valle2_amd/csrc/vh_common.h b/valle2_amd/csrc/vh_common.h
--- a/valle2_amd/csrc/vh_common.h
+++ b/valle2_amd/csrc/vh_common.h
@@ -79,6 +79,9 @@
 
 int vh_tuning(int knob);
 
+void vh_internal_set_all_eos_word(int32_t* word);
+int32_t* vh_internal_all_eos_word(void);
+
 template <int CTRL, int ROW_MASK>
 __device__ __forceinline__ float dpp_get(float v, float identity) {
     return __int_as_float(__builtin_amdgcn_update_dpp(__float_as_int(identity), __float_as_int(v), CTRL,
@@ -115,6 +118,12 @@
     return __builtin_nontemporal_load(reinterpret_cast<const f32x4*>(p));
 }
 __device__ __forceinline__ void st4(float* p, f32x4 v) { *reinterpret_cast<f32x4*>(p) = v; }
+
+__device__ __forceinline__ void vh_count_eos(int32_t* eos_count, int step, int rows, int32_t* word) {
+    const int before = atomicAdd(&eos_count[step], 1);
+    if (word && before + 1 == rows && __hip_atomic_load(word, __ATOMIC_RELAXED, __HIP_MEMORY_SCOPE_SYSTEM) < 0)
+        __hip_atomic_store(word, step, __ATOMIC_RELAXED, __HIP_MEMORY_SCOPE_SYSTEM);
+}
 
 __device__ __forceinline__ float vh_exp2(float x) { return __builtin_amdgcn_exp2f(x); }
 
diff --git a/valle2_amd/engine.py b/valle2_amd/engine.py
--- a/valle2_amd/engine.py
+++ b/valle2_amd/engine.py
@@ -296,9 +296,12 @@
 
 
 def transformer_forward(transformer, x, cache: KVCache, *, mode, x_len=0, x_len_dev=None,
-                        kv_len=None, mask=None, pad=None, embedding=None, scratch=None, x_in=None):
+                        kv_len=None, mask=None, pad=None, embedding=None, scratch=None, x_in=None, last_rows=None):
     cfg = transformer.hparams
     B, T, d = x.shape
+    if last_rows is not None and (d != cfg.n_heads * HEAD_DIM or last_rows.dtype != torch.int32 or last_rows.numel() != B
+                                  or not last_rows.is_cuda or not last_rows.is_contiguous()):
+        raise _lib.VhError('last_rows: a contiguous int32 device tensor (B), head width 64')
     if not x.is_contiguous():
         raise _lib.VhError('x must be contiguous')
     if x_in is not None and (tuple(x_in.shape) != tuple(x.shape) or x_in.dtype != torch.float32):
@@ -322,8 +325,12 @@
         x_len_dev=ptr(x_len_dev), kv_len=ptr(kv_len), mask=ptr(mask), pad=ptr(pad),
         x=ptr(x), xn=ptr(scratch.xn), q=ptr(scratch.q), attn=ptr(scratch.attn),
         hidden=ptr(scratch.hidden), gemm_ws=ptr(scratch.ws), gemm_ws_bytes=scratch.ws_bytes, x_in=ptr(x_in))
+    last_out = None
+    if last_rows is not None:
+        last_out = torch.empty(B, d, device=x.device, dtype=torch.float32)
+        desc.last_rows, desc.last_out = ptr(last_rows), ptr(last_out)
     check(_lib.lib().vh_transformer_forward(C.byref(desc), stream()), 'vh_transformer_forward')
-    return x
+    return x if last_out is None else last_out
 
 
 def _transformer_forward_generic(transformer, x, *, mode, x_len, x_len_dev, kv_len, mask, pad, embedding, x_in, cache=None):
@@ -650,6 +657,7 @@
         self.sampling = self.sampling[:3] + (int(seed),)
         if self.seed_dev is not None:
             self.seed_dev.copy_(torch.tensor([int(seed)], dtype=torch.int64), non_blocking=True)
+        check(_lib.lib().vh_ar_decoder_rearm(self._h), 'vh_ar_decoder_rearm')
 
     def capture(self):
         if self.use_graph and not self._captured:
@@ -670,6 +678,24 @@
             for _ in range(n_steps):
                 check(L.vh_ar_decoder_step(self._h, s), 'vh_ar_decoder_step')
 
+    def sample_from(self, hidden_last, rows=slice(None), cache_len=None):
+        if rows != slice(None) or not self._captured:
+            return super().sample_from(hidden_last, rows, cache_len)
+        L = _lib.lib()
+        check(L.vh_ar_decoder_word_scope(self._h, 1), 'vh_ar_decoder_word_scope')
+        try:
+            super().sample_from(hidden_last, rows, cache_len)
+        finally:
+            L.vh_ar_decoder_word_scope(self._h, 0)
+
+    def run_until_eos(self, max_steps):
+        if max_steps <= 0:
+            return 0, None
+        self.capture()
+        ran, stop = C.c_int(0), C.c_int(-1)
+        check(_lib.lib().vh_ar_decoder_run(self._h, max_steps, stream(), C.byref(ran), C.byref(stop)), 'vh_ar_decoder_run')
+        return ran.value, (stop.value if stop.value >= 0 else None)
+
     def profile_attn(self, n_steps):
         ms, floor, kern = C.c_float(0), C.c_float(0), C.c_float(0)
         check(_lib.lib().vh_ar_decoder_profile_attn(self._h, n_steps, stream(), C.byref(ms), C.byref(floor),
diff --git a/valle2_amd/generation.py b/valle2_amd/generation.py
--- a/valle2_amd/generation.py
+++ b/valle2_amd/generation.py
@@ -15,6 +15,8 @@
 from .utils import get_best_beam
 
 EOS_POLL = 32
+EOS_RUN = os.environ.get('VALLE2_EOS_RUN', '1') != '0'
+PROMPT_TAIL = os.environ.get('VALLE2_PROMPT_TAIL', '1') != '0'
 MAX_DECODE_ROWS = 64
 SHARED_PROMPT = os.environ.get('VALLE2_SHARED_PROMPT', '1') != '0'
 _DECODER_ENV = ('VALLE2_HEAD_FUSED', 'VALLE2_SHARED_SPLIT', 'VALLE2_FOLD_LN', 'VALLE2_DECODE_W16')
@@ -324,6 +326,7 @@
             model._embed_rows(texts[b].unsqueeze(0), codes[b * n:b * n + 1, :plan.pls[b]], x[b:b + 1])
         fwd = dict(x_len_dev=torch.tensor(plan.txs, **i32), kv_len=torch.tensor(plan.ctx, **i32))
     into = state.cache if state.prefix is None else state.prefix
+    last = None
     if plan.prefill_bf16:
         transformer_forward_bf16(model.transformer, x, into, mode=kernels.MASK_PREFIX,
                                  scratch=ForwardScratch16(rows * s0, d, cfg.dim_feedforward, dev), **fwd)
@@ -334,8 +337,14 @@
         wide.narrow_into(state.prefix)
     else:
         scratch = None if plan.kind in (RECOMPUTE_GENERAL, ROWS_HD) else ForwardScratch(rows * s0, d, cfg.dim_feedforward, dev)
-        transformer_forward(model.transformer, x, into, mode=kernels.MASK_PREFIX, scratch=scratch, **fwd)
-    if plan.ragged:
+        if PROMPT_TAIL and plan.kind in (ROWS, SHARED, GROUPED):
+            last_rows = (fwd['kv_len'] - 1) if plan.ragged else torch.full((rows,), s0 - 1, **i32)
+            last = transformer_forward(model.transformer, x, into, mode=kernels.MASK_PREFIX, scratch=scratch, last_rows=last_rows, **fwd)
+        else:
+            transformer_forward(model.transformer, x, into, mode=kernels.MASK_PREFIX, scratch=scratch, **fwd)
+    if last is not None:
+        last = last.expand(B, d) if plan.kind == SHARED else last
+    elif plan.ragged:
         last = x[torch.arange(plan.G, device=dev), fwd['kv_len'].long() - 1]
     elif plan.kind == SHARED:
         last = x[:, -1].expand(B, d)
@@ -394,6 +403,8 @@
 
 
 def _decode_cached(plan, dec, done):
+    if dec.use_graph and EOS_RUN and _lib.TUNING.get(_lib.TUNE_EOS_RUN, 0) != 1:
+        return done + dec.run_until_eos(plan.max_new - done)[0], None
     while done < plan.max_new:
         n = min(EOS_POLL, plan.max_new - done)
         dec.run(n)
```

Measured after the change: 49450 tokens/s, median of 6. About the same (+0.6%).
